# DakeQQ/Text-to-Speech-TTS-ONNX

Measured on AMD Instinct MI355X. Metric: audio_seconds_per_second, higher is better.
Workload: dtype f32

## Files before the change

text-to-speech-tts-onnx_amd/csrc/capi.hip:

```cpp
#include "common.h"
#include "bigvgan.h"
#include "f5.h"
#include "gpt.h"
#include "gpt_pick.h"
#include "cond.h"
#include <algorithm>
#include <mutex>
#include <exception>

using namespace mi;

struct mi_bigvgan { BigVGAN* impl; std::mutex mu; };
struct mi_f5 { F5* impl; std::mutex mu; };
struct mi_gpt { Gpt* impl; std::mutex mu; };
struct mi_cond { Cond* impl; std::mutex mu; };

template <typename F> static int guard(F&& f, bool exclusive = false) {
    try {
        options_init();
        std::shared_lock<std::shared_mutex> rd(option_lock(), std::defer_lock);
        std::unique_lock<std::shared_mutex> wr(option_lock(), std::defer_lock);
        if (exclusive) wr.lock(); else rd.lock();
        f();
        return MI_OK;
// ... 122 lines not shown

int mi_bigvgan_forward_latent(mi_bigvgan* h, const float* latent, int T_codes, const float* conds, int64_t n_conds,
                              int16_t* out, float* out_f32, int mem) {
    return guard([&] {
        MI_REQUIRE(h && h->impl, "mi_bigvgan_forward_latent: null handle");
        std::lock_guard<std::mutex> lk_(h->mu);
        MI_REQUIRE(mem == MI_HOST || mem == MI_DEVICE, "mi_bigvgan_forward_latent: bad mem kind");
        h->impl->run_latent(latent, T_codes, conds, (long)n_conds, out_f32, out, mem);
    });
}

static std::vector<int> bigvgan_lengths(const int64_t* lens, int B, int64_t lo, const char* what) {
    MI_REQUIRE(lens && B >= 1, what);
    std::vector<int> v(B);
    for (int b = 0; b < B; ++b) {
        MI_REQUIRE(lens[b] >= lo && lens[b] < (1L << 30), what);
        v[b] = (int)lens[b];
    }
    return v;
}

int mi_bigvgan_forward_ragged(mi_bigvgan* h, int B, const float* mel, const int64_t* frames, int16_t* out_i16, float* out_f32,
                              int64_t out_cap, int64_t* out_lens, int mem) {
    return guard([&] {
        MI_REQUIRE(h && h->impl, "mi_bigvgan_forward_ragged: null handle");
        std::lock_guard<std::mutex> lk_(h->mu);
        MI_REQUIRE(mem == MI_HOST || mem == MI_DEVICE, "mi_bigvgan_forward_ragged: bad mem kind");
        MI_REQUIRE(out_i16, "mi_bigvgan_forward_ragged: null out_i16");
        const std::vector<int> F = bigvgan_lengths(frames, B, 1, "mi_bigvgan_forward_ragged: B >= 1 items of >= 1 frames");
        h->impl->run_ragged(mel, B, F.data(), out_f32, out_i16, (long)out_cap, out_lens, mem);
    });
}

int mi_bigvgan_forward_latent_ragged(mi_bigvgan* h, int B, const float* latent, const int64_t* t_codes, const float* conds,
                                     int64_t n_conds, int16_t* out_i16, float* out_f32, int64_t out_cap, int64_t* out_lens, int mem) {
    return guard([&] {
        MI_REQUIRE(h && h->impl, "mi_bigvgan_forward_latent_ragged: null handle");
        std::lock_guard<std::mutex> lk_(h->mu);
        MI_REQUIRE(mem == MI_HOST || mem == MI_DEVICE, "mi_bigvgan_forward_latent_ragged: bad mem kind");
        MI_REQUIRE(out_i16, "mi_bigvgan_forward_latent_ragged: null out_i16");
        const std::vector<int> T = bigvgan_lengths(t_codes, B, 3, "mi_bigvgan_forward_latent_ragged: B >= 1 items of >= 3 latent rows");
        h->impl->run_latent_ragged(latent, B, T.data(), conds, (long)n_conds, out_f32, out_i16, (long)out_cap, out_lens, mem);
    });
}

int mi_aa_activation1d(const float* x, int B, int C, int T, const float* alpha_log, const float* beta_log,
                       int logscale, int post, int dtype, float* y) {
    return guard([&] {
        MI_REQUIRE(x && y && alpha_log && beta_log && B > 0 && C > 0 && T > 0, "mi_aa_activation1d: bad arguments");
        unit_aa_activation1d(x, B, C, T, alpha_log, beta_log, logscale, post, dtype, y);
    });
}

int mi_aa_conv1d(const float* x, int B, int C, int T, const float* alpha_log, const float* beta_log, int logscale,
                 const float* w, const float* bias, int k, int dilation, const float* res, int dtype, float* y) {
    return guard([&] {
        MI_REQUIRE(x && y && w && bias && alpha_log && beta_log && B > 0 && C > 0 && T > 0 && k > 0 && (k & 1) && dilation > 0,
                   "mi_aa_conv1d: bad arguments");
        unit_aa_conv1d(x, B, C, T, alpha_log, beta_log, logscale, w, bias, k, dilation, res, dtype, 1, y);
    });
}

int mi_conv1d(const float* x, int B, int Cin, int T, const float* w, const float* bias, int Cout, int k, int dilation,
              int padding, int groups, int dtype, float* y) {
    return guard([&] {
        MI_REQUIRE(x && w && y && B > 0 && Cin > 0 && Cout > 0 && T > 0 && k > 0 && dilation > 0 && groups > 0 && padding >= 0,
                   "mi_conv1d: bad arguments");
        unit_conv1d(x, B, Cin, T, w, bias, Cout, k, dilation, padding, groups, dtype, y);
    });
}

int mi_conv_transpose1d(const float* x, int B, int Cin, int T, const float* w, const float* bias, int Cout, int k,
                        int stride, int padding, int dtype, float* y) {
    return guard([&] {
        MI_REQUIRE(x && w && y && B > 0 && Cin > 0 && Cout > 0 && T > 0, "mi_conv_transpose1d: bad arguments");
        unit_conv_transpose1d(x, B, Cin, T, w, bias, Cout, k, stride, padding, dtype, y);
    });
}

int64_t mi_f5_param_count(const int32_t* cfg_i, int n_i, const float* cfg_f, int n_f) {
    int64_t n = -1;
    int rc = guard([&] { n = f5_param_count(parse_f5_cfg(cfg_i, n_i, cfg_f, n_f)); });
    return rc == MI_OK ? n : (int64_t)rc;
}

mi_f5* mi_f5_create(const int32_t* cfg_i, int n_i, const float* cfg_f, int n_f, const float* weights, int64_t n_weights,
                    int dtype, int device) {
    mi_f5* h = nullptr;
    int rc = guard([&] {
        MI_REQUIRE(weights != nullptr, "mi_f5_create: null weights");
        F5Cfg c = parse_f5_cfg(cfg_i, n_i, cfg_f, n_f);
        F5* impl = new F5(c, weights, n_weights, dtype, device);
        h = new mi_f5; h->impl = impl;
    });
    return rc == MI_OK ? h : nullptr;
}

mi_f5* mi_f5_create_mem(const int32_t* cfg_i, int n_i, const float* cfg_f, int n_f, const float* weights, int64_t n_weights,
                        int dtype, int device, int mem) {
    mi_f5* h = nullptr;
    int rc = guard([&] {
        MI_REQUIRE(weights != nullptr && (mem == MI_HOST || mem == MI_DEVICE), "mi_f5_create_mem: null weights / bad mem kind");
        F5Cfg c = parse_f5_cfg(cfg_i, n_i, cfg_f, n_f);
        F5* impl = new F5(c, weights, n_weights, dtype, device, mem);
        h = new mi_f5; h->impl = impl;
    });
    return rc == MI_OK ? h : nullptr;
}

void mi_f5_destroy(mi_f5* h) {
    if (!h) return;
    delete h->impl;
    delete h;
}

struct F5Recover {
    F5* e; int n;
    explicit F5Recover(F5* e_) : e(e_), n(std::uncaught_exceptions()) {}
    ~F5Recover() { if (std::uncaught_exceptions() > n) e->recover(); }
};
#define F5_CHECK(h, mem, name)                                                     \
    MI_REQUIRE((h) && (h)->impl, name ": null handle");                            \
    std::lock_guard<std::mutex> lk_((h)->mu);                                      \
    F5Recover rec_((h)->impl);                                                     \
    ArithScope arith_((h)->impl->arith);                                           \
    MI_REQUIRE((mem) == MI_HOST || (mem) == MI_DEVICE, name ": bad mem kind")

static void copy_out(void* dst, const void* src, size_t bytes, int mem, hipStream_t s) {
    if (!dst) return;
    MI_HIP(hipMemcpyAsync(dst, src, bytes, mem == MI_HOST ? hipMemcpyDeviceToHost : hipMemcpyDeviceToDevice, s));
}

int mi_f5_tables(mi_f5* h, float* time_expand, float* delta_t) {
    return guard([&] {
        MI_REQUIRE(h && h->impl, "mi_f5_tables: null handle");
        std::lock_guard<std::mutex> lk_(h->mu);
        F5& e = *h->impl;
        if (time_expand) std::memcpy(time_expand, e.h_time_expand.data(), e.h_time_expand.size() * 4);
        if (delta_t) std::memcpy(delta_t, e.h_delta.data(), e.h_delta.size() * 4);
    });
}

int64_t mi_f5_info(mi_f5* h, const char* key) {
    int64_t v = -1;
    int rc = guard([&] {
        MI_REQUIRE(h && h->impl && key, "mi_f5_info: null handle / key");
        std::lock_guard<std::mutex> lk_(h->mu);
        F5& e = *h->impl;
        ArithScope as(e.arith);
        const std::string k(key);
        if (k == "f32_arithmetic") v = e.dtype != MI_F32 ? -1 : !gemm_x3_enabled() ? ARITH_NATIVE : (gemm_x3p_enabled() ? e.np : ARITH_BF16X3);
        else if (k == "saturation_events") v = e.sat_events;
        else if (k == "adaln_fold") v = (e.fold_built && e.cfg.ln_fold != 0) ? 1 : 0;
        else if (k == "attn_v_rows") v = attention_kv_layout(0, e.dtype, true).v_rows;
        else MI_REQUIRE(false, "mi_f5_info: unknown key");
    });
    return rc == MI_OK ? v : (int64_t)rc;
}

int mi_f5_preprocess(mi_f5* h, const int16_t* audio, int64_t L, const int32_t* text_ids, int64_t T, int64_t max_duration,
                     const float* noise_in, uint64_t seed, float* noise, float* rope_cos, float* rope_sin,
                     float* cat_mel_text, float* cat_mel_text_drop, int64_t* ref_signal_len, int mem) {
    return guard([&] {
        F5_CHECK(h, mem, "mi_f5_preprocess");
        F5& e = *h->impl;
        MI_REQUIRE(max_duration > 0 && max_duration <= e.cfg.max_len && T >= 0 && T < (1 << 20) && L > 0 && L < (1L << 31),
                   "mi_f5_preprocess: sizes");
        const int N = (int)max_duration;
        const int R = e.preprocess(1, audio, L, text_ids, (int)T, N, noise_in, seed, mem);
        hipStream_t s = e.stream;
        const size_t cd = e.cfg.cond_dim(), D = e.cfg.dim_head;
        copy_out(noise, e.d_noise.p, (size_t)N * e.cfg.mel * 4, mem, s);
        copy_out(rope_cos, e.rope_cos.p, (size_t)N * D * 4, mem, s);
        copy_out(rope_sin, e.rope_sin.p, (size_t)N * D * 4, mem, s);
        copy_out(cat_mel_text, e.d_cmt.p, (size_t)N * cd * 4, mem, s);
        copy_out(cat_mel_text_drop, e.d_cmtd.p, (size_t)N * cd * 4, mem, s);
        MI_HIP(hipStreamSynchronize(s));
        e.finish_call();
        if (ref_signal_len) *ref_signal_len = R;
    });
}

int mi_f5_transformer_step(mi_f5* h, float* noise, const float* cmt, const float* cmtd, int U, int64_t N,
                           int32_t* time_step, int fuse, int mem) {
    return guard([&] {
        F5_CHECK(h, mem, "mi_f5_transformer_step");
        MI_REQUIRE(noise && cmt && cmtd && time_step && fuse >= 1 && U >= 1 && N > 0, "mi_f5_transformer_step: bad arguments");
        F5& e = *h->impl;
        f5_run_checked(e, [&] {
            e.load_cond(noise, cmt, cmtd, U, (int)N, mem);
            e.build_cat_cond(U, (int)N);
            e.steps(U, (int)N, *time_step, fuse);
            MI_HIP(hipStreamSynchronize(e.stream));
        });
        copy_out(noise, e.d_noise.p, (size_t)U * N * e.cfg.mel * 4, mem, e.stream);
        MI_HIP(hipStreamSynchronize(e.stream));
        e.finish_call();
        *time_step += fuse;
    });
}

int mi_f5_sample(mi_f5* h, float* noise, const float* cmt, const float* cmtd, int U, int64_t N, int k0, int n_steps, int mem) {
    return guard([&] {
        F5_CHECK(h, mem, "mi_f5_sample");
        MI_REQUIRE(noise && cmt && cmtd && U >= 1 && N > 0, "mi_f5_sample: bad arguments");
        F5& e = *h->impl;
        f5_run_checked(e, [&] {
            e.load_cond(noise, cmt, cmtd, U, (int)N, mem);
            e.build_cat_cond(U, (int)N);
            e.steps(U, (int)N, k0, n_steps);
            MI_HIP(hipStreamSynchronize(e.stream));
        });
        copy_out(noise, e.d_noise.p, (size_t)U * N * e.cfg.mel * 4, mem, e.stream);
        MI_HIP(hipStreamSynchronize(e.stream));
        e.finish_call();
    });
}

int mi_f5_dit_eval(mi_f5* h, const float* noise, const float* cmt, const float* cmtd, int U, int64_t N, int k, float* pred, int mem) {
    return guard([&] {
        F5_CHECK(h, mem, "mi_f5_dit_eval");
        MI_REQUIRE(noise && cmt && cmtd && pred && U >= 1 && N > 0, "mi_f5_dit_eval: bad arguments");
        F5& e = *h->impl;
        f5_run_checked(e, [&] {
            e.load_cond(noise, cmt, cmtd, U, (int)N, mem);
            e.build_cat_cond(U, (int)N);
            e.dit_eval(U, (int)N, k);
            MI_HIP(hipStreamSynchronize(e.stream));
        });
        copy_out(pred, e.pred_rows(U, (int)N), (size_t)2 * U * N * e.cfg.mel * 4, mem, e.stream);
        MI_HIP(hipStreamSynchronize(e.stream));
        e.finish_call();
    });
}

int mi_f5_decode(mi_f5* h, const float* denoised, int U, int64_t N, int64_t ref_signal_len, int16_t* out, float* out_f32,
                 int64_t* out_len, int mem) {
    return guard([&] {
        F5_CHECK(h, mem, "mi_f5_decode");
        MI_REQUIRE(denoised && (out || out_f32) && U >= 1 && N > 0 && ref_signal_len >= 0 && ref_signal_len < N,
                   "mi_f5_decode: bad arguments");
        F5& e = *h->impl;
        e.load_cond(denoised, nullptr, nullptr, U, (int)N, mem);
        const long len = e.decode(e.d_noise.as<float>(), U, (int)N, (int)ref_signal_len, out_f32 ? e.v_outf.as<float>() : nullptr,
                                  out ? e.v_outi.as<int16_t>() : nullptr);
        copy_out(out, e.v_outi.p, (size_t)U * len * 2, mem, e.stream);
        copy_out(out_f32, e.v_outf.p, (size_t)U * len * 4, mem, e.stream);
        MI_HIP(hipStreamSynchronize(e.stream));
        e.finish_call();
        if (out_len) *out_len = len;
    });
}

int mi_f5_synthesize(mi_f5* h, int U, const int16_t* audio, int64_t L, const int32_t* text_ids, int64_t T,
                     int64_t max_duration, const float* noise_in, uint64_t seed, int16_t* out, int64_t* out_len, int mem) {
    return guard([&] {
        F5_CHECK(h, mem, "mi_f5_synthesize");
        MI_REQUIRE(audio && text_ids && out && U >= 1 && max_duration > 0, "mi_f5_synthesize: bad arguments");
        F5& e = *h->impl;
        const int N = (int)max_duration;
        long len = 0;
        f5_run_checked(e, [&] {
            const int R = e.preprocess(U, audio, L, text_ids, (int)T, N, noise_in, seed, mem);
            e.build_cat_cond(U, N);
            e.steps(U, N, 0, e.cfg.nfe - 1);
            len = e.decode(e.d_noise.as<float>(), U, N, R, nullptr, e.v_outi.as<int16_t>());
            copy_out(out, e.v_outi.p, (size_t)U * len * 2, mem, e.stream);
            MI_HIP(hipStreamSynchronize(e.stream));
        });
        e.finish_call();
        if (out_len) *out_len = len;
    });
}

int mi_f5_synthesize_mel(mi_f5* h, int U, const int16_t* audio, int64_t L, const int32_t* text_ids, int64_t T,
                         int64_t max_duration, const float* noise_in, uint64_t seed, float* mel_out, int64_t* n_frames, int mem) {
    return guard([&] {
        F5_CHECK(h, mem, "mi_f5_synthesize_mel");
        MI_REQUIRE(audio && text_ids && mel_out && U >= 1 && max_duration > 0, "mi_f5_synthesize_mel: bad arguments");
        F5& e = *h->impl;
        const int N = (int)max_duration;
        int F = 0;
        f5_run_checked(e, [&] {
            const int R = e.preprocess(U, audio, L, text_ids, (int)T, N, noise_in, seed, mem);
            const int mel = e.cfg.mel;
            F = N - R;
            MI_REQUIRE(F >= 1, "mi_f5_synthesize_mel: max_duration leaves no generated frames");
            e.build_cat_cond(U, N);
            e.steps(U, N, 0, e.cfg.nfe - 1);
            float* dst = mel_out;
            if (mem == MI_HOST) { e.v_outf.ensure((size_t)U * mel * F * 4); dst = e.v_outf.as<float>(); }
            for (int u = 0; u < U; ++u)
                launch_nlc_to_ncl(e.d_noise.as<float>() + ((size_t)u * N + R) * mel, dst + (size_t)u * mel * F, 1, mel, F, MI_F32, e.stream);
            if (mem == MI_HOST) copy_out(mel_out, dst, (size_t)U * mel * F * 4, mem, e.stream);
            MI_HIP(hipStreamSynchronize(e.stream));
        });
        e.finish_call();
        if (n_frames) *n_frames = F;
    });
}

static std::vector<int> f5_lengths(const int64_t* lens, int U, int64_t lo, int64_t hi, const char* what) {
    MI_REQUIRE(lens && U >= 1, what);
    std::vector<int> v(U);
    for (int u = 0; u < U; ++u) {
        MI_REQUIRE(lens[u] >= lo && lens[u] <= hi, what);
// ... 930 lines not shown
```

text-to-speech-tts-onnx_amd/csrc/common.h:

```cpp
#pragma once
#include <hip/hip_runtime.h>
#include <hip/hip_fp16.h>
#include <cstdint>
#include <cstdio>
#include <cstring>
#include <cmath>
#include <string>
#include <vector>
#include <stdexcept>
#include <map>
#include <shared_mutex>

#include "../../include/mi355tts.h"
#include "options.h"

namespace mi {

struct Error : std::runtime_error {
    int code;
    Error(int c, const std::string& m) : std::runtime_error(m), code(c) {}
};
void set_last_error(const std::string& m);

#define MI_HIP(expr)                                                                              \
    do {                                                                                          \
        hipError_t _e = (expr);                                                                   \
        if (_e != hipSuccess)                                                                     \
            throw mi::Error(MI_EHIP, std::string(#expr) + ": " + hipGetErrorString(_e) + " @" +   \
                                         __FILE__ + ":" + std::to_string(__LINE__));              \
    } while (0)

#define MI_REQUIRE(cond, msg)                                                                     \
    do {                                                                                          \
        if (!(cond)) throw mi::Error(MI_EINVAL, std::string(msg) + " [" #cond "]");               \
    } while (0)

using f16 = _Float16;
using bf16 = __bf16;
typedef unsigned int u32x4 __attribute__((ext_vector_type(4)));

template <typename T> struct DT;
template <> struct DT<float> { static constexpr int id = MI_F32; };
template <> struct DT<f16>   { static constexpr int id = MI_F16; };
template <> struct DT<bf16>  { static constexpr int id = MI_BF16; };

inline size_t dtype_size(int dt) { return dt == MI_F32 ? 4 : 2; }

template <typename T> __host__ __device__ inline float to_f32(T v) { return (float)v; }
template <typename T> __host__ __device__ inline T from_f32(float v) { return (T)v; }

struct DevBuf {
    void* p = nullptr;
    size_t bytes = 0;
    DevBuf() = default;
    DevBuf(const DevBuf&) = delete;
    DevBuf& operator=(const DevBuf&) = delete;
    DevBuf(DevBuf&& o) noexcept : p(o.p), bytes(o.bytes) { o.p = nullptr; o.bytes = 0; }
    DevBuf& operator=(DevBuf&& o) noexcept {
        if (this != &o) { release(); p = o.p; bytes = o.bytes; o.p = nullptr; o.bytes = 0; }
        return *this;
    }
    ~DevBuf() { release(); }
    void release() { if (p) { (void)hipFree(p); p = nullptr; bytes = 0; } }
    void ensure(size_t n) {
        if (n <= bytes) return;
        release();
        MI_HIP(hipMalloc(&p, n));
        bytes = n;
    }
    template <typename T> T* as() const { return reinterpret_cast<T*>(p); }
};

void upload_as(DevBuf& dst, const float* src, size_t n, int dt, hipStream_t s);
void upload_f32(DevBuf& dst, const float* src, size_t n, hipStream_t s);
int device_cus();

struct BlobReader {
    int mem; hipStream_t s;
    std::vector<std::vector<float>> keep;
    BlobReader(int mem_, hipStream_t s_) : mem(mem_), s(s_) {}
    const float* host(const float* p, size_t n);
    void put(DevBuf& dst, const float* p, size_t n, int dt, size_t dst_off = 0);
};

struct ProfScope {
    int fam; hipStream_t s; hipEvent_t e0 = nullptr, e1 = nullptr; bool on; double bytes_ = 0, flops_ = 0;
    ProfScope(int family, hipStream_t stream, double bytes, double flops);
    ~ProfScope();
};
enum { FAM_CONV_GEMM = 0, FAM_AA = 1, FAM_CONV_POST = 2, FAM_ATTN = 3, FAM_NORM = 4, FAM_OTHER = 5, FAM_COUNT = 6 };
void prof_set_kernel(const char* expr, const char* t = nullptr, const char* to = nullptr);
void prof_kernel_suffix(const char* sfx);
template <typename T> inline const char* type_label();
template <> inline const char* type_label<float>() { return "float"; }
template <> inline const char* type_label<f16>() { return "_Float16"; }
template <> inline const char* type_label<bf16>() { return "__bf16"; }
#define MI_LAUNCH(K, T_, TO_, grid, blk, lds, s, ...)                                                  \
    do {                                                                                               \
        mi::prof_set_kernel(#K, mi::type_label<T_>(), mi::type_label<TO_>());                          \
        hipLaunchKernelGGL(K, grid, blk, lds, s, __VA_ARGS__);                                         \
    } while (0)
void prof_collect();
unsigned prof_mask();

enum Act { ACT_NONE = 0, ACT_GELU_TANH = 1, ACT_GELU_ERF = 2, ACT_MISH = 3, ACT_SILU = 4 };
enum EpiMode { EPI_PLAIN = 0, EPI_CONVT = 1, EPI_QKV_ROPE = 2 };

struct ConvGemm {
    int dtype = MI_F32;
    int out_dtype = -1;
    const void* x = nullptr;
    const void* w = nullptr;
    const float* bias = nullptr;
    void* out = nullptr;
    const void* res = nullptr;
    const float* gate = nullptr;
    long gate_bstride = 0;
    int B = 1, G = 1;
    int T_in = 0;
    int M = 0, N = 0, Cin = 0, taps = 1, dil = 1, pad = 0;
    long x_bstride = 0, x_rstride = 0;
    long out_bstride = 0, out_rstride = 0;
    long x_goff = 0;
    int act = ACT_NONE;
    float alpha = 1.f;
    int accumulate = 0;
    int epi = EPI_PLAIN;
    int u = 1, Cout = 0, padT = 0, T_out = 0;
    const float* rope_cos = nullptr; const float* rope_sin = nullptr; int heads = 0, head_dim = 0;
    const void* rope_pack = nullptr;
    void* out2 = nullptr; void* out3 = nullptr;
    int rows_per_item = 0;
    int m_off = 0;
    long v_ld = 0;
    int kv_planes = 0; long k_ld = 0;
    int v_rows = 0;
    float* sk_ws = nullptr; int* sk_flags = nullptr; int sk_slots = 0;
    const void* w3 = nullptr;
    const void* xp = nullptr; const void* w3p = nullptr; int np = 3;
    const void* gcp_w = nullptr;
    void* out_planes = nullptr;
    const float* ln_scale = nullptr; void* ln_out = nullptr; float* ln_stats_out = nullptr; int ln_out_np = 0;
    const float* ln_stats_in = nullptr; const float* ln_p = nullptr; const float* ln_c = nullptr; int ln_dim = 0; float ln_eps = 0.f;
    int ln_final = 0;
    int* sat = nullptr;
    const int* lens = nullptr; int len_mul = 1, len_add = 0;
};
constexpr int LN_BLK = 32;
void launch_conv_gemm(const ConvGemm& p, hipStream_t s);
bool gemm_ln_fold_ok(const ConvGemm& p);
constexpr int X3P_PLANE = 128 * 32 * 2;
constexpr int X3P_CHUNK = 3 * X3P_PLANE;
__host__ __device__ inline int x3p_chunk_bytes(int np) { return np * X3P_PLANE; }
__host__ __device__ inline long x3p_slot_offset(long row, int s8, int nch, int np = 3) {
    const int r = (int)(row & 127);
    return ((row >> 7) * nch + (s8 >> 2)) * (long)(np * X3P_PLANE) + r * 64 + (((s8 & 3) ^ ((r >> 2) & 3)) << 4);
}
long x3p_bytes(long rows, long K, int np = 3);
void x3p_split_rows(const float* x, long ld, void* planes, int rows, int K, hipStream_t s, int np = 3, int* sat = nullptr);
size_t gconv_pairs_planes_bytes(int G, int taps);
void gconv_pairs_split_weights(const float* w, void* wp, int G, int taps, hipStream_t s);
size_t gconv16_image_bytes(int G, int taps);
void gconv16_build_weights(const void* w, int dtype, void* img, int G, int taps, hipStream_t s);
int x3p_planes();
bool gemm_x3p_enabled();
bool gemm_x3p_would_run(const ConvGemm& p);
bool gemm_x3p_can_write_planes(const ConvGemm& p);
struct SkWorkspace {
    DevBuf ws, flags; int slots = 0;
    void ensure(int n_slots, hipStream_t s);
    void reset(hipStream_t s);
    bool tripped() const;
    void attach(ConvGemm& g) const { g.sk_ws = ws.as<float>(); g.sk_flags = flags.as<int>(); g.sk_slots = slots; }
};

struct ArithOverride {
    int gemm_x3 = -1;
    int gemm_x3p = -1;
    int planes = -1;
    int n64_pairs = -1;
    int gconv = -1;
    int attn_x3 = -1;
    int attn_np = -1;
};
enum { ARITH_DEFAULT = -1, ARITH_NATIVE = 0, ARITH_PAIRS = 2, ARITH_BF16X3 = 3 };
ArithOverride arith_for(int kind);
ArithOverride& arith_tls();
struct ArithScope {
    ArithOverride saved;
    explicit ArithScope(const ArithOverride& a) : saved(arith_tls()) { arith_tls() = a; }
    ~ArithScope() { arith_tls() = saved; }
    ArithScope(const ArithScope&) = delete;
    ArithScope& operator=(const ArithScope&) = delete;
};

struct AAAct {
    int dtype = MI_F32;
    const void* x = nullptr; void* y = nullptr;
    const float* alpha = nullptr;
    const float* inv_beta = nullptr;
    int B = 1, T = 0, C = 0;
    int post = 0;
    const int* lens = nullptr; int len_mul = 1, len_add = 0;
};
void launch_aa_act(const AAAct& p, hipStream_t s);
const float* aa_filter_host();

struct AAConv {
    int dtype = MI_F32;
    const void* x = nullptr; const void* w = nullptr;
    const float* bias = nullptr;
    const float* snake_alpha = nullptr; const float* snake_inv_beta = nullptr;
    void* out = nullptr; const void* res = nullptr;
    int B = 1, T = 0, C = 0, k = 3, dil = 1;
    float alpha = 1.f; int accumulate = 0;
    const int* lens = nullptr; int len_mul = 1, len_add = 0;
};
void launch_aa_conv(const AAConv& p, hipStream_t s);
void split3_planes(const float* w, void* planes, long n, hipStream_t s);
bool gemm_x3_enabled();

void launch_ncl_to_nlc(const float* x, void* y, int B, int C, int T, int Cpad, int dtype, hipStream_t s);
void launch_ncl_to_nlc_len(const float* x, void* y, int B, int C, int T, int Cpad, int dtype, const int* lens, const long* offs,
                           hipStream_t s);
void launch_nlc_to_ncl(const void* x, float* y, int B, int C, int T, int dtype, hipStream_t s);
void launch_conv_post(const void* x, const float* w , float bias, int B, int T, int C, int dtype,
                      int use_tanh, float* out_f32, int16_t* out_i16, hipStream_t s);
void launch_conv_post_len(const void* x, const float* w, float bias, int B, int T, int C, int dtype, int use_tanh, float* out_f32,
                          int16_t* out_i16, const int* lens, int len_mul, int len_add, const long* offs, hipStream_t s);

}
```

text-to-speech-tts-onnx_amd/csrc/f5.h:

```cpp
#pragma once
#include <algorithm>

#include "common.h"
#include "f5_kernels.h"

namespace mi {

struct F5Cfg {
    int dim, depth, heads, dim_head, ff_mult, mel, text_dim, vocab, conv_layers, conv_mult, pos_k, pos_g, freq_dim,
        nfe, max_len, n_fft, hop, sr, vd, vi, vlayers;
    float cfg_strength, sway;
    float score_scale = 1.f;
    int f32_arith = ARITH_DEFAULT;
    int mel_type = 0;
    int ln_fold = -1;
    int ff() const { return dim * ff_mult; }
    int nb() const { return n_fft / 2 + 1; }
    int cat_dim() const { return 2 * mel + text_dim; }
    int cond_dim() const { return mel + text_dim; }
};
F5Cfg parse_f5_cfg(const int32_t* ci, int ni, const float* cf, int nf);
int64_t f5_param_count(const F5Cfg& c);

struct Lin { DevBuf w, b, w3, w3p; int n = 0, k = 0; };

struct F5 {
    F5Cfg cfg;
    int dtype, device;
    hipStream_t stream = nullptr;

    Lin in_proj, gconv1, gconv2, proj_out;
    Lin proj_out_k; int proj_parts = 1; DevBuf pred_sum;
    const float* pred_rows(int U, int N);
    int cat_pad = 0;
    int cat_ld() const { return cfg.cat_dim() + cat_pad; }
    struct Block { Lin qkv, o, ff1, ff2; };
    std::vector<Block> blocks;
    DevBuf mod;
    long mod_ld = 0;
    DevBuf delta_t;
    DevBuf rope_cos, rope_sin;
    DevBuf rope_pack;
    std::vector<float> h_time_expand, h_delta;

    DevBuf text_emb, text_pos, stft_w, fbank;
    struct TextBlock { DevBuf dw_w, dw_b, ln_w, ln_b, grn_g, grn_b; Lin pw1, pw2; };
    std::vector<TextBlock> tblocks;

    Lin v_embed, v_head, istft;
    DevBuf v_norm_w, v_norm_b, v_fnorm_w, v_fnorm_b, wsi;
    struct VBlock { DevBuf dw_w, dw_b, n_w, n_b; Lin pw1, pw2; };
    std::vector<VBlock> vblocks;

    struct GraphEntry { hipGraphExec_t exec = nullptr; int uses = 0; };
    std::map<std::vector<int>, GraphEntry> graphs;
    bool use_graph = true;
    long graph_epoch = 0;
    void drop_graphs();
    void recover();
    void steps_eager(int U, int N, int k0, int nsteps, const int* lens = nullptr);

    SkWorkspace sk;
    DevBuf attn_ws, attn_cnt;
    long attn_ws_floats = 0, attn_cnt_n = 0;
    int ws_U = 0, ws_N = 0;
    int np = 3;
    ArithOverride arith;
    int arith_kind = ARITH_DEFAULT;
    DevBuf Ap, Ap2;
    int ap2_cols() const { return std::max(cfg.ff(), cat_ld()); }
    bool fold_built = false;
    DevBuf ApN;
    DevBuf ln_stats;
    DevBuf ln_fin;
    DevBuf ln_tab;
    long ln_ld = 0, ln_blk = 0;
    DevBuf d_sat;
    long sat_events = 0;
    void build_ln_tables(int i, DevBuf& G, DevBuf& S, DevBuf& tmpw);
    void set_arith(int kind);
    bool take_saturation();
    void finish_call();
    DevBuf d_noise, d_cmt, d_cmtd, cat, h32, hT, c1, X, Ub, qb, kb, vb, Ob, Hff, pred;
    DevBuf p_audio, p_pad, p_spec, p_mag, p_mel, p_ids, p_tid, p_err, p_tx, p_ty, p_ty2, p_ss;
    std::vector<float> h_noise;
    DevBuf v_h, v_z, v_z2, v_s, v_c, v_fr, v_outf, v_outi;

    F5(const F5Cfg& c, const float* w, int64_t nw, int dt, int dev, int mem = MI_HOST);
    ~F5();
    void ensure_workspace(int U, int N);
    void gemm(int dt, const void* x, long xb, long xr, int K, const Lin& L, void* out, int odt, long ob, long orr,
              int B, int M, int act = ACT_NONE, const void* res = nullptr, const float* gate = nullptr);
    int preprocess(int U, const int16_t* audio, long L, const int32_t* text_ids, int T, int N,
                   const float* noise_in, uint64_t seed, int mem);
    void stft(const int16_t* audio_dev, int U, long L, int pad = -1);
    void check_text_ids();
    void load_cond(const float* noise, const float* cmt, const float* cmtd, int U, int N, int mem);
    void build_cat_cond(int U, int N);
    void dit_eval(int U, int N, int k, const int* lens = nullptr);
    void steps(int U, int N, int k0, int nsteps, const int* lens = nullptr);
    DevBuf d_len;
    std::vector<int> h_len;
    int ref_frames(long L) const;
    const int* set_lengths(int U, const int* lens);
    void zero_pad_rows_cond(int U, int Nmax, const int* lens);
    void preprocess_ragged(int U, const int16_t* audio, const long* L, const int32_t* text_ids, const int* T, const int* Ns, int Nmax,
                           const float* noise_in, uint64_t seed, int mem, int* R);
    long decode(const float* denoised_dev, int U, int N, int R, float* out_f, int16_t* out_i);
};

}
```

text-to-speech-tts-onnx_amd/csrc/f5.hip:

```cpp
#include "f5.h"

namespace mi {

static int rup(int a, int b) { return (a + b - 1) / b * b; }

F5Cfg parse_f5_cfg(const int32_t* ci, int ni, const float* cf, int nf) {
    MI_REQUIRE(ci && ni >= 21 && ni <= 24 && cf && (nf == 2 || nf == 3),
               "f5 cfg: expected 21 ints (+ up to 3 optional: fp32 arithmetic, mel type, AdaLN fold) + 2 floats (+ the optional attention score scale)");
    F5Cfg c;
    int i = 0;
    c.dim = ci[i++]; c.depth = ci[i++]; c.heads = ci[i++]; c.dim_head = ci[i++]; c.ff_mult = ci[i++]; c.mel = ci[i++];
    c.text_dim = ci[i++]; c.vocab = ci[i++]; c.conv_layers = ci[i++]; c.conv_mult = ci[i++]; c.pos_k = ci[i++];
    c.pos_g = ci[i++]; c.freq_dim = ci[i++]; c.nfe = ci[i++]; c.max_len = ci[i++]; c.n_fft = ci[i++]; c.hop = ci[i++];
    c.sr = ci[i++]; c.vd = ci[i++]; c.vi = ci[i++]; c.vlayers = ci[i++];
    if (ni > 21) c.f32_arith = ci[21];
    if (ni > 22) c.mel_type = ci[22];
    if (ni > 23) c.ln_fold = ci[23];
    MI_REQUIRE(c.f32_arith == ARITH_DEFAULT || c.f32_arith == ARITH_NATIVE || c.f32_arith == ARITH_PAIRS || c.f32_arith == ARITH_BF16X3,
               "f5 cfg: fp32 arithmetic is -1 (process default), 0 (native fp32 MFMA), 2 (fp16 pairs) or 3 (three bf16 planes)");
    MI_REQUIRE((c.mel_type == 0 || c.mel_type == 1) && c.ln_fold >= -1 && c.ln_fold <= 1, "f5 cfg: mel type is 0 (vocos) or 1 (bigvgan); AdaLN fold is -1, 0 or 1");
    c.cfg_strength = cf[0]; c.sway = cf[1];
    if (nf == 3) { c.score_scale = cf[2]; MI_REQUIRE(c.score_scale > 0.f && c.score_scale <= 1e4f, "f5 cfg: attention score scale"); }
    MI_REQUIRE(c.dim == c.heads * c.dim_head, "f5 cfg: dim != heads*dim_head");
    MI_REQUIRE(c.dim_head == 64, "f5: the attention kernel is built for head_dim 64");
    MI_REQUIRE(c.dim % 32 == 0 && c.dim <= 2048 && c.text_dim % 8 == 0 && c.mel % 4 == 0, "f5 cfg: widths");
    MI_REQUIRE(c.dim % c.pos_g == 0 && (c.dim / c.pos_g) % 8 == 0 && c.pos_k % 2 == 1, "f5 cfg: pos conv");
    MI_REQUIRE(c.nfe >= 2 && c.nfe <= 1024 && c.max_len >= 16 && c.depth > 0, "f5 cfg: sampler");
    MI_REQUIRE(c.n_fft % 8 == 0 && c.n_fft % c.hop == 0 && c.vd % 4 == 0 && c.vi % 4 == 0 && c.vd <= 2048, "f5 cfg: vocoder");
    MI_REQUIRE(c.freq_dim % 2 == 0 && c.conv_mult >= 1 && c.text_dim * c.conv_mult <= 4096, "f5 cfg: text");
    return c;
}

int64_t f5_param_count(const F5Cfg& c) {
    const int64_t d = c.dim, td = c.text_dim, ff = c.ff(), ti = td * c.conv_mult, cin = c.cat_dim();
    int64_t n = d * c.freq_dim + d + d * d + d;
    n += (int64_t)(c.vocab + 1) * td;
    n += (int64_t)c.conv_layers * (td * 7 + td + td + td + ti * td + ti + ti + ti + td * ti + td);
    n += d * cin + d + 2 * (d * (d / c.pos_g) * c.pos_k + d);
    n += (int64_t)c.depth * (6 * d * d + 6 * d + 4 * (d * d + d) + ff * d + ff + d * ff + d);
    n += 2 * d * d + 2 * d + (int64_t)c.mel * d + c.mel;
    const int64_t vd = c.vd, vi = c.vi;
    n += vd * c.mel * 7 + vd + 2 * vd;
    n += (int64_t)c.vlayers * (vd * 7 + vd + 2 * vd + vi * vd + vi + vd * vi + vd);
    n += 2 * vd + (int64_t)(c.n_fft + 2) * vd + (c.n_fft + 2);
    return n;
}

static void up_lin(Lin& L, const float* w, const float* b, int n, int k, int dt, hipStream_t s) {
    L.n = n; L.k = k;
    upload_as(L.w, w, (size_t)n * k, dt, s);
    if (b) upload_f32(L.b, b, n, s);
}
static void put_lin(BlobReader& R, Lin& L, const float* w, const float* b, int n, int k, int dt) {
    L.n = n; L.k = k;
    R.put(L.w, w, (size_t)n * k, dt);
    if (b) R.put(L.b, b, n, MI_F32);
}
static std::vector<float> relayout(const float* w, int Co, int Ci, int k) {
    std::vector<float> o((size_t)Co * k * Ci);
    for (int co = 0; co < Co; ++co)
        for (int ci = 0; ci < Ci; ++ci)
            for (int j = 0; j < k; ++j) o[((size_t)co * k + j) * Ci + ci] = w[((size_t)co * Ci + ci) * k + j];
    return o;
}
static inline float siluf(float v) { return v / (1.f + expf(-v)); }
static inline float round_f16(float v) { return (float)(f16)v; }

F5::F5(const F5Cfg& c, const float* w, int64_t nw, int dt, int dev, int mem) : cfg(c), dtype(dt), device(dev) {
    arith_kind = dt == MI_F32 ? c.f32_arith : ARITH_DEFAULT;
    arith = arith_for(arith_kind);
    ArithScope arith_scope(arith);
    np = x3p_planes();
    MI_REQUIRE(dt == MI_F32 || dt == MI_F16 || dt == MI_BF16, "f5: bad dtype");
    MI_REQUIRE(c.score_scale == 1.f || dt == MI_F16, "f5: the attention score scale (reference fp16-transformer form) needs an f16 engine");
    MI_REQUIRE(nw == f5_param_count(c), "f5: weight blob size does not match the config");
    MI_HIP(hipSetDevice(dev));
    MI_HIP(hipStreamCreateWithFlags(&stream, hipStreamNonBlocking));
    use_graph = !env_first_is("MI355TTS_NO_GRAPH", '1');
    hipStream_t s = stream;
    d_sat.ensure(64);
    MI_HIP(hipMemsetAsync(d_sat.p, 0, 64, s));
    const int d = c.dim, td = c.text_dim, ff = c.ff(), ti = td * c.conv_mult, cin = c.cat_dim();
    if (dt == MI_F32 && !env_first_is("MI355TTS_CAT_PAD", '0')) cat_pad = rup(cin, 64) - cin;
    const float* p = w;
    auto take = [&](size_t n) { const float* r = p; p += n; return r; };
    BlobReader R(mem, s);

    const float* tw0 = R.host(take((size_t)d * c.freq_dim), (size_t)d * c.freq_dim); const float* tb0 = R.host(take(d), d);
    const float* tw2 = R.host(take((size_t)d * d), (size_t)d * d); const float* tb2 = R.host(take(d), d);
    const int steps = c.nfe, half = c.freq_dim / 2;
    std::vector<float> ts(steps);
    for (int i = 0; i < steps; ++i) {
        const float t = (float)i / (float)(steps - 1);
        ts[i] = t + c.sway * (cosf(3.14159265358979323846f * 0.5f * t) - 1.f + t);
    }
    h_delta.resize(steps - 1);
    for (int i = 0; i + 1 < steps; ++i) h_delta[i] = ts[i + 1] - ts[i];
    upload_f32(delta_t, h_delta.data(), steps - 1, s);
    h_time_expand.assign((size_t)steps * d, 0.f);
    {
        const float ef = logf(10000.f) / (float)(half - 1);
        std::vector<float> emb(c.freq_dim), hid(d);
        for (int i = 0; i < steps; ++i) {
            for (int j = 0; j < half; ++j) {
                const float a = ts[i] * (1000.0f * expf((float)j * -ef));
                emb[j] = sinf(a); emb[half + j] = cosf(a);
            }
            for (int o = 0; o < d; ++o) {
                float acc = tb0[o];
                for (int j = 0; j < c.freq_dim; ++j) acc += tw0[(size_t)o * c.freq_dim + j] * emb[j];
                hid[o] = siluf(acc);
            }
            for (int o = 0; o < d; ++o) {
                float acc = tb2[o];
                for (int j = 0; j < d; ++j) acc += tw2[(size_t)o * d + j] * hid[j];
                h_time_expand[(size_t)i * d + o] = acc;
            }
        }
    }
    R.put(text_emb, take((size_t)(c.vocab + 1) * td), (size_t)(c.vocab + 1) * td, MI_F32);
    {
        std::vector<float> pos((size_t)c.max_len * td);
        std::vector<float> fr(td / 2);
        for (int j = 0; j < td / 2; ++j) fr[j] = 1.0f / powf(10000.0f, (float)(2 * j) / (float)td);
        for (int n = 0; n < c.max_len; ++n)
            for (int j = 0; j < td / 2; ++j) {
                const float a = (float)n * fr[j];
                pos[(size_t)n * td + j] = cosf(a); pos[(size_t)n * td + td / 2 + j] = sinf(a);
            }
        upload_f32(text_pos, pos.data(), pos.size(), s);
    }
    tblocks.resize(c.conv_layers);
    for (auto& tb : tblocks) {
        R.put(tb.dw_w, take((size_t)td * 7), (size_t)td * 7, MI_F32);
        R.put(tb.dw_b, take(td), td, MI_F32);
        R.put(tb.ln_w, take(td), td, MI_F32);
        R.put(tb.ln_b, take(td), td, MI_F32);
        const float* w1 = take((size_t)ti * td); const float* b1 = take(ti);
        put_lin(R, tb.pw1, w1, b1, ti, td, MI_F32);
        R.put(tb.grn_g, take(ti), ti, MI_F32);
        R.put(tb.grn_b, take(ti), ti, MI_F32);
        const float* w2 = take((size_t)td * ti); const float* b2 = take(td);
        put_lin(R, tb.pw2, w2, b2, td, ti, MI_F32);
    }
    {
        const float* pw = take((size_t)d * cin); const float* pb = take(d);
        if (cat_ld() == cin) put_lin(R, in_proj, pw, pb, d, cin, dt);
        else {
            const int kp = cat_ld();
            const float* hw = R.host(pw, (size_t)d * cin); const float* hb = R.host(pb, d);
            std::vector<float> wp((size_t)d * kp, 0.f);
            for (int o = 0; o < d; ++o) std::copy(hw + (size_t)o * cin, hw + (size_t)(o + 1) * cin, wp.begin() + (size_t)o * kp);
            up_lin(in_proj, wp.data(), hb, d, kp, dt, s);
        }
        const int cg = d / c.pos_g;
        const size_t gw = (size_t)d * cg * c.pos_k;
        const float* w1 = R.host(take(gw), gw); const float* b1 = R.host(take(d), d);
        auto r1 = relayout(w1, d, cg, c.pos_k);
        up_lin(gconv1, r1.data(), b1, d, cg * c.pos_k, dt, s);
        const float* w2 = R.host(take(gw), gw); const float* b2 = R.host(take(d), d);
        auto r2 = relayout(w2, d, cg, c.pos_k);
        up_lin(gconv2, r2.data(), b2, d, cg * c.pos_k, dt, s);
        if (dt != MI_F32 && cg == 64 && c.pos_k >= 8 && c.pos_k <= 127) {
            for (Lin* L : {&gconv1, &gconv2}) {
                L->w3p.ensure(gconv16_image_bytes(c.pos_g, c.pos_k));
                gconv16_build_weights(L->w.p, dt, L->w3p.p, c.pos_g, c.pos_k, s);
            }
        }
        if (dt == MI_F32 && cg == 64 && c.pos_k >= 8 && c.pos_k <= 127) {
            for (Lin* L : {&gconv1, &gconv2}) {
                L->w3p.ensure(gconv_pairs_planes_bytes(c.pos_g, c.pos_k));
                gconv_pairs_split_weights(L->w.as<float>(), L->w3p.p, c.pos_g, c.pos_k, s);
            }
        }
    }
    mod_ld = (long)c.depth * 6 * d + 2 * d;
    mod.ensure((size_t)steps * mod_ld * 4);
    DevBuf d_silu_t, d_tmpw, d_tmpb;
    {
        std::vector<float> st(h_time_expand.size());
        for (size_t i = 0; i < st.size(); ++i) st[i] = siluf(h_time_expand[i]);
        upload_f32(d_silu_t, st.data(), st.size(), s);
    }
    auto mod_gemm = [&](const float* mw, const float* mb, int n, long col) {
        R.put(d_tmpw, mw, (size_t)n * d, MI_F32);
        R.put(d_tmpb, mb, n, MI_F32);
        ConvGemm g;
        g.dtype = MI_F32; g.x = d_silu_t.p; g.w = d_tmpw.p; g.bias = d_tmpb.as<float>(); g.out = mod.as<float>() + col;
        g.B = 1; g.T_in = steps; g.M = steps; g.N = n; g.Cin = d; g.x_rstride = d; g.x_bstride = (long)steps * d;
        g.out_rstride = mod_ld; g.out_bstride = (long)steps * mod_ld;
        launch_conv_gemm(g, s);
        MI_HIP(hipStreamSynchronize(s));
    };
    blocks.resize(c.depth);
    for (int i = 0; i < c.depth; ++i) {
        Block& bk = blocks[i];
        const float* mw = take((size_t)6 * d * d); const float* mb = take((size_t)6 * d);
        mod_gemm(mw, mb, 6 * d, (long)i * 6 * d);
        bk.qkv.n = 3 * d; bk.qkv.k = d;
        bk.qkv.w.ensure((size_t)3 * d * d * dtype_size(dt)); bk.qkv.b.ensure((size_t)3 * d * 4);
        for (int t3 = 0; t3 < 3; ++t3) {
            const float* wt = take((size_t)d * d); const float* bt = take(d);
            if (t3 == 0) { R.put(bk.qkv.w, wt, (size_t)d * d, dt, 0); R.put(bk.qkv.b, bt, d, MI_F32, 0); }
            else { R.put(bk.qkv.w, wt, (size_t)d * d, dt, (size_t)t3 * d * d); R.put(bk.qkv.b, bt, d, MI_F32, (size_t)t3 * d); }
        }
        const float* wo = take((size_t)d * d); const float* bo = take(d);
        put_lin(R, bk.o, wo, bo, d, d, dt);
        const float* w1 = take((size_t)ff * d); const float* b1 = take(ff);
        put_lin(R, bk.ff1, w1, b1, ff, d, dt);
        const float* w2 = take((size_t)d * ff); const float* b2 = take(d);
        put_lin(R, bk.ff2, w2, b2, d, ff, dt);
        if (dt == MI_F32) {
            for (Lin* L : {&bk.qkv, &bk.o, &bk.ff1, &bk.ff2}) {
                L->w3.ensure((size_t)3 * L->n * L->k * 2);
                split3_planes(L->w.as<float>(), L->w3.p, (long)L->n * L->k, s);
                launch_absmax(L->w.as<float>(), (long)L->n * L->k, d_sat.as<unsigned>() + 1, s);
            }
        }
    }
    if (dt == MI_F32) {
        unsigned bits = 0;
        MI_HIP(hipMemcpyAsync(&bits, d_sat.as<unsigned>() + 1, 4, hipMemcpyDeviceToHost, s));
        MI_HIP(hipStreamSynchronize(s));
        float wmax; std::memcpy(&wmax, &bits, 4);
        int kind = arith_kind;
        if (np == 2 && gemm_x3p_enabled() && !(wmax < 65504.f)) kind = ARITH_BF16X3;
        set_arith(kind);
    }
    fold_built = false;
    const bool want_fold = c.ln_fold != 0;
    if (want_fold && d >= 1024 && d % 128 == 0 && ff % 64 == 0) {
        ln_blk = (long)6 * d + 2 * ff;
        ln_ld = (long)c.depth * ln_blk;
        ln_tab.ensure((size_t)steps * ln_ld * 4);
        DevBuf G, S, tmpw;
        G.ensure((size_t)steps * d * 4); S.ensure((size_t)steps * d * 4);
        if (dt != MI_F32) tmpw.ensure((size_t)std::max(3 * d, ff) * d * 4);
        for (int i = 0; i < c.depth; ++i) build_ln_tables(i, G, S, tmpw);
        MI_HIP(hipStreamSynchronize(s));
        fold_built = true;
    }
    {
        const float* mw = take((size_t)2 * d * d); const float* mb = take((size_t)2 * d);
        mod_gemm(mw, mb, 2 * d, (long)c.depth * 6 * d);
        const float* pw = take((size_t)c.mel * d); const float* pb = take(c.mel);
        put_lin(R, proj_out, pw, pb, c.mel, d, dt);
        {
            const int parts = (int)env_int("MI355TTS_PROJ_PARTS", 4);
            if (dt == MI_F32 && parts > 1 && parts <= 8 && d % (parts * 32) == 0) {
                proj_parts = parts;
                const int kq = d / parts;
                const float* hw = R.host(pw, (size_t)c.mel * d); const float* hb = R.host(pb, c.mel);
                std::vector<float> wq((size_t)c.mel * d), bq((size_t)parts * c.mel, 0.f);
                for (int q = 0; q < parts; ++q)
                    for (int o = 0; o < c.mel; ++o)
                        std::copy(hw + (size_t)o * d + (size_t)q * kq, hw + (size_t)o * d + (size_t)(q + 1) * kq, wq.begin() + ((size_t)q * c.mel + o) * kq);
                std::copy(hb, hb + c.mel, bq.begin());
                up_lin(proj_out_k, wq.data(), bq.data(), parts * c.mel, kq, dt, s);
            }
        }
    }
    {
        const int D = c.dim_head;
        std::vector<float> rc((size_t)c.max_len * D), rs((size_t)c.max_len * D);
        for (int n = 0; n < c.max_len; ++n)
            for (int j = 0; j < D / 2; ++j) {
                const float inv = 1.0f / powf(10000.0f, (float)(2 * j) / (float)D);
                const float a = (float)n * inv;
                const float cc = round_f16(cosf(a)), ss = round_f16(sinf(a));
                rc[(size_t)n * D + 2 * j] = rc[(size_t)n * D + 2 * j + 1] = cc;
                rs[(size_t)n * D + 2 * j] = rs[(size_t)n * D + 2 * j + 1] = ss;
            }
        upload_f32(rope_cos, rc.data(), rc.size(), s);
        upload_f32(rope_sin, rs.data(), rs.size(), s);
        std::vector<f16> pk((size_t)c.max_len * D);
        for (int n = 0; n < c.max_len; ++n)
            for (int j = 0; j < D / 2; ++j) {
                pk[(size_t)n * D + 2 * j] = (f16)rc[(size_t)n * D + 2 * j];
                pk[(size_t)n * D + 2 * j + 1] = (f16)rs[(size_t)n * D + 2 * j];
            }
        rope_pack.ensure(pk.size() * sizeof(f16));
        MI_HIP(hipMemcpyAsync(rope_pack.p, pk.data(), pk.size() * sizeof(f16), hipMemcpyHostToDevice, s));
        MI_HIP(hipStreamSynchronize(s));
    }
    {
        const int nf = c.n_fft, nb = c.nb();
        std::vector<float> win(nf);
        const float wstep = (float)(2.0 * M_PI / nf);
        for (int n = 0; n < nf; ++n) win[n] = cosf((float)n * wstep) * -0.5f + 0.5f;
        std::vector<float> sw((size_t)2 * nb * nf);
        const float two_pi = (float)(2.0 * M_PI);
        for (int f = 0; f < nb; ++f)
            for (int t = 0; t < nf; ++t) {
                const float om = ((two_pi * (float)f) * (float)t) / (float)nf;
                sw[(size_t)f * nf + t] = cosf(om) * win[t];
                sw[(size_t)(nb + f) * nf + t] = -sinf(om) * win[t];
            }
        if (c.mel_type == 1) {
            for (int f = 0; f < nb; ++f)
                for (int t = 0; t < nf; ++t) {
                    const double om = 2.0 * M_PI * (double)((long)f * t % nf) / nf;
                    sw[(size_t)f * nf + t] = (float)(std::cos(om) * (double)win[t]);
                    sw[(size_t)(nb + f) * nf + t] = (float)(-std::sin(om) * (double)win[t]);
                }
        }
        upload_f32(stft_w, sw.data(), sw.size(), s);
        const int ldm = rup(nb, 8);
        std::vector<float> fb((size_t)c.mel * ldm, 0.f);
        if (c.mel_type == 1) {
            const double f_sp = 200.0 / 3, min_log_hz = 1000.0, logstep = std::log(6.4) / 27.0, min_log_mel = min_log_hz / f_sp;
            auto h2m = [&](double f) { return f < min_log_hz ? f / f_sp : min_log_mel + std::log(f / min_log_hz) / logstep; };
            auto m2h = [&](double m) { return m < min_log_mel ? f_sp * m : min_log_hz * std::exp(logstep * (m - min_log_mel)); };
            const double m0 = h2m(0.0), m1 = h2m((double)c.sr / 2);
            std::vector<double> mf(c.mel + 2);
            for (int i = 0; i < c.mel + 2; ++i) mf[i] = m2h(m0 + (m1 - m0) * i / (c.mel + 1));
            for (int m = 0; m < c.mel; ++m) {
                const double enorm = 2.0 / (mf[m + 2] - mf[m]);
                for (int k = 0; k < nb; ++k) {
                    const double fr = (double)c.sr / 2 * k / (nb - 1);
                    const double lower = (fr - mf[m]) / (mf[m + 1] - mf[m]), upper = (mf[m + 2] - fr) / (mf[m + 2] - mf[m + 1]);
                    fb[(size_t)m * ldm + k] = (float)(std::max(0.0, std::min(lower, upper)) * enorm);
                }
            }
        }
        const double m_min = 0.0, m_max = 2595.0 * std::log10(1.0 + (c.sr / 2) / 700.0);
        std::vector<double> fpts(c.mel + 2);
        for (int i = 0; i < c.mel + 2; ++i) {
            const double m = m_min + (m_max - m_min) * i / (c.mel + 1);
            fpts[i] = 700.0 * (std::pow(10.0, m / 2595.0) - 1.0);
        }
        for (int k = 0; k < nb && c.mel_type == 0; ++k) {
            const double fr = (double)(c.sr / 2) * k / (nb - 1);
            for (int m = 0; m < c.mel; ++m) {
                const double down = (fr - fpts[m]) / (fpts[m + 1] - fpts[m]);
                const double up = (fpts[m + 2] - fr) / (fpts[m + 2] - fpts[m + 1]);
                fb[(size_t)m * ldm + k] = (float)std::max(0.0, std::min(down, up));
            }
        }
        upload_f32(fbank, fb.data(), fb.size(), s);
        const int kp = rup(2 * nb, 4);
        std::vector<float> ib((size_t)nf * kp, 0.f);
        for (int n = 0; n < nf; ++n)
            for (int k = 0; k < nb; ++k) {
                const double sc = ((k == 0 || k == nb - 1) ? 1.0 : 2.0) / nf * ((double)c.hop / nf) * (double)win[n];
                const double ang = 2.0 * M_PI * (double)k * (double)n / nf;
                ib[(size_t)n * kp + k] = (float)(sc * std::cos(ang));
                ib[(size_t)n * kp + nb + k] = (float)(sc * -std::sin(ang));
            }
        istft.n = nf; istft.k = kp;
        upload_f32(istft.w, ib.data(), ib.size(), s);
        const size_t wl = (size_t)nf + (size_t)c.hop * (c.max_len - 1);
        std::vector<float> ws(wl, 0.f);
        float wmax = 0.f;
        for (int n = 0; n < nf; ++n) wmax = std::max(wmax, fabsf(win[n]));
        std::vector<float> wsq(nf);
        for (int n = 0; n < nf; ++n) { const float wn = win[n] / wmax; wsq[n] = wn * wn; }
        for (int i = 0; i < c.max_len; ++i)
            for (int n = 0; n < nf; ++n) ws[(size_t)i * c.hop + n] += wsq[n];
        for (size_t i = 0; i < wl; ++i) ws[i] = (float)nf / (ws[i] * (float)c.hop + 1e-7f);
        upload_f32(wsi, ws.data(), wl, s);
    }
    {
        const int vd = c.vd, vi = c.vi;
        const size_t ewn = (size_t)vd * c.mel * 7;
        const float* ew = R.host(take(ewn), ewn); const float* eb = R.host(take(vd), vd);
        auto re = relayout(ew, vd, c.mel, 7);
        up_lin(v_embed, re.data(), eb, vd, c.mel * 7, MI_F32, s);
        R.put(v_norm_w, take(vd), vd, MI_F32); R.put(v_norm_b, take(vd), vd, MI_F32);
        vblocks.resize(c.vlayers);
        for (auto& vb_ : vblocks) {
            R.put(vb_.dw_w, take((size_t)vd * 7), (size_t)vd * 7, MI_F32); R.put(vb_.dw_b, take(vd), vd, MI_F32);
            R.put(vb_.n_w, take(vd), vd, MI_F32); R.put(vb_.n_b, take(vd), vd, MI_F32);
            const float* w1 = take((size_t)vi * vd); const float* b1 = take(vi);
            put_lin(R, vb_.pw1, w1, b1, vi, vd, MI_F32);
            const float* w2 = take((size_t)vd * vi); const float* b2 = take(vd);
            put_lin(R, vb_.pw2, w2, b2, vd, vi, MI_F32);
        }
        R.put(v_fnorm_w, take(vd), vd, MI_F32); R.put(v_fnorm_b, take(vd), vd, MI_F32);
        const float* hw = take((size_t)(c.n_fft + 2) * vd); const float* hb = take(c.n_fft + 2);
        put_lin(R, v_head, hw, hb, c.n_fft + 2, vd, MI_F32);
    }
    MI_HIP(hipStreamSynchronize(s));
    MI_REQUIRE(p - w == nw, "f5: weight walk mismatch");
}

F5::~F5() {
    drop_graphs();
    if (stream) (void)hipStreamDestroy(stream);
}

void F5::set_arith(int kind) {
    arith_kind = kind;
    arith = arith_for(kind);
    ArithScope sc(arith);
    np = x3p_planes();
    drop_graphs();
    if (dtype != MI_F32) return;
    const bool planes = gemm_x3p_enabled();
    auto build_planes = [&](Lin* L) {
        if (!planes || L->n % 128 != 0 || L->k % 32 != 0) { L->w3p.release(); return; }
        L->w3p.ensure((size_t)x3p_bytes(L->n, L->k, np));
        x3p_split_rows(L->w.as<float>(), L->k, L->w3p.p, L->n, L->k, stream, np);
    };
    for (Block& bk : blocks)
        for (Lin* L : {&bk.qkv, &bk.o, &bk.ff1, &bk.ff2}) build_planes(L);
    build_planes(&in_proj);
    if (ws_U > 0) {
        const long rows = (long)2 * ws_U * ws_N;
        Ap.ensure((size_t)x3p_bytes(rows, cfg.dim, np)); Ap2.ensure((size_t)x3p_bytes(rows, ap2_cols(), np)); ApN.ensure((size_t)x3p_bytes(rows, cfg.dim, np));
    }
    MI_HIP(hipStreamSynchronize(stream));
}

void F5::build_ln_tables(int i, DevBuf& G, DevBuf& S, DevBuf& tmpw) {
    const int d = cfg.dim, ff = cfg.ff(), steps = cfg.nfe;
    Block& bk = blocks[i];
    float* tab = ln_tab.as<float>() + (size_t)i * ln_blk;
    auto run = [&](const Lin& L, long col_shift, long col_scale, float* out_p, float* out_c) {
        launch_ln_gather(mod.as<float>(), mod_ld, (long)i * 6 * d + col_scale, (long)i * 6 * d + col_shift, G.as<float>(), S.as<float>(), steps, d, stream);
        const float* w32 = L.w.as<float>();
        if (dtype != MI_F32) { launch_cast_to_f32(L.w.p, dtype, tmpw.as<float>(), (long)L.n * L.k, stream); w32 = tmpw.as<float>(); }
        ConvGemm g;
        g.dtype = MI_F32; g.x = G.p; g.w = w32; g.bias = nullptr; g.out = out_p;
        g.B = 1; g.T_in = steps; g.M = steps; g.N = L.n; g.Cin = d; g.x_rstride = d; g.x_bstride = (long)steps * d;
        g.out_rstride = ln_ld; g.out_bstride = (long)steps * ln_ld;
        launch_conv_gemm(g, stream);
        g.x = S.p; g.bias = L.b.as<float>(); g.out = out_c;
        launch_conv_gemm(g, stream);
        MI_HIP(hipStreamSynchronize(stream));
    };
    run(bk.qkv, 0, d, tab, tab + 3 * d);
    run(bk.ff1, 3 * d, 4 * d, tab + 6 * d, tab + 6 * d + ff);
}

bool F5::take_saturation() {
    if (!d_sat.p) return false;
    int flag = 0;
    MI_HIP(hipMemcpy(&flag, d_sat.p, 4, hipMemcpyDeviceToHost));
    if (!flag) return false;
    MI_HIP(hipMemset(d_sat.p, 0, 4));
    return true;
}

void F5::finish_call() {
    check_text_ids();
}

void F5::ensure_workspace(int U, int N) {
    if (U <= ws_U && N <= ws_N) return;
    drop_graphs();
    const int Um = std::max(U, ws_U), Nm = std::max(N, ws_N);
    const F5Cfg& c = cfg;
    const size_t es = dtype_size(dtype);
    const size_t rows = (size_t)2 * Um * Nm;
    sk.ensure(1024, stream);
    {
        if (ATTN_WS_TILES > attn_cnt_n) {
            attn_ws_floats = ATTN_WS_TILES * ATTN_MAX_SLICES * ATTN_SLOT_SPLIT;
            attn_ws.ensure((size_t)attn_ws_floats * 4);
            attn_cnt.ensure((size_t)ATTN_WS_TILES * 4);
            MI_HIP(hipMemsetAsync(attn_cnt.p, 0, (size_t)ATTN_WS_TILES * 4, stream));
            attn_cnt_n = ATTN_WS_TILES;
        }
    }
    d_noise.ensure((size_t)Um * Nm * c.mel * 4);
    d_cmt.ensure((size_t)Um * Nm * c.cond_dim() * 4);
    d_cmtd.ensure((size_t)Um * Nm * c.cond_dim() * 4);
    if (rows * cat_ld() * es > cat.bytes) {
        cat.ensure(rows * cat_ld() * es);
        if (cat_ld() != c.cat_dim()) MI_HIP(hipMemsetAsync(cat.p, 0, cat.bytes, stream));
    }
    h32.ensure(rows * c.dim * 4); hT.ensure(rows * c.dim * es); c1.ensure(rows * c.dim * es);
    X.ensure(rows * c.dim * 4); Ub.ensure(rows * c.dim * es);
    qb.ensure(rows * c.dim * es); Ob.ensure(rows * c.dim * es);
    {
        const size_t keypad = (size_t)(Nm + 63) / 64 * 64;
        size_t kbytes = rows * c.dim * es, vbytes = (size_t)2 * Um * (size_t)(Nm + 8) * c.dim * es;
        if (dtype == MI_F32) { kbytes = std::max(kbytes, (size_t)2 * Um * keypad * c.dim * 6); vbytes = std::max(vbytes, (size_t)2 * Um * keypad * c.dim * 6); }
        if (kbytes > kb.bytes) { kb.ensure(kbytes); MI_HIP(hipMemsetAsync(kb.p, 0, kbytes, stream)); }
        if (vbytes > vb.bytes) { vb.ensure(vbytes); MI_HIP(hipMemsetAsync(vb.p, 0, vbytes, stream)); }
    }
    Hff.ensure(rows * c.ff() * es);
    if (dtype == MI_F32) {
        Ap.ensure((size_t)x3p_bytes((long)rows, c.dim, np)); Ap2.ensure((size_t)x3p_bytes((long)rows, ap2_cols(), np));
        if (fold_built) ApN.ensure((size_t)x3p_bytes((long)rows, c.dim, np));
    }
    if (fold_built) { ln_stats.ensure((rows + 128) * (size_t)(c.dim / LN_BLK) * 2 * 4); if (dtype != MI_F32) ln_fin.ensure((rows + 128) * 8); }
    pred.ensure(rows * c.mel * 4 * proj_parts);
    if (proj_parts > 1) pred_sum.ensure(rows * c.mel * 4);
    const int ti = c.text_dim * c.conv_mult;
    p_ids.ensure((size_t)Um * Nm * 4);
    p_tx.ensure((size_t)2 * Um * Nm * c.text_dim * 4); p_ty.ensure((size_t)2 * Um * Nm * c.text_dim * 4);
    p_ty2.ensure((size_t)2 * Um * Nm * ti * 4); p_ss.ensure((size_t)2 * Um * ti * 4);
    const size_t fr = (size_t)Um * Nm;
    v_h.ensure(fr * c.vd * 4); v_z.ensure(fr * c.vd * 4); v_z2.ensure(fr * c.vi * 4);
    v_s.ensure(fr * (c.n_fft + 2) * 4); v_c.ensure(fr * istft.k * 4); v_fr.ensure(fr * c.n_fft * 4);
    v_outf.ensure(fr * c.hop * 4); v_outi.ensure(fr * c.hop * 2);
    ws_U = Um; ws_N = Nm;
}

void F5::gemm(int dt, const void* x, long xb, long xr, int K, const Lin& L, void* out, int odt, long ob, long orr, int B,
              int M, int act, const void* res, const float* gate) {
    ConvGemm g;
    g.dtype = dt; g.out_dtype = odt; g.x = x; g.w = L.w.p; g.w3 = L.w3.p; g.bias = L.b.p ? L.b.as<float>() : nullptr; g.out = out;
    g.res = res; g.gate = gate; g.gate_bstride = 0;
    g.B = B; g.T_in = M; g.M = M; g.N = L.n; g.Cin = K; g.taps = 1;
    g.x_bstride = xb; g.x_rstride = xr; g.out_bstride = ob; g.out_rstride = orr; g.act = act;
    g.sat = d_sat.as<int>();
    sk.attach(g);
    if (B > 1 && xb == (long)M * xr && ob == (long)M * orr) {
        g.B = 1; g.T_in = B * M; g.M = B * M;
    }
    if (dt == MI_F32 && L.w3p.p && g.B == 1 && Ap.p && gemm_x3p_enabled()) {
        DevBuf& ab = K <= cfg.dim ? Ap : Ap2;
        g.xp = ab.p; g.w3p = L.w3p.p; g.np = np;
        if (gemm_x3p_would_run(g)) {
            MI_REQUIRE(x3p_bytes(g.M, K, np) <= (long)ab.bytes, "F5::gemm: the panel planes of the rows do not fit their buffer");
            x3p_split_rows((const float*)x, xr, const_cast<void*>(g.xp), g.M, K, stream, np, d_sat.as<int>());
        } else {
            g.xp = nullptr; g.w3p = nullptr;
        }
    }
    launch_conv_gemm(g, stream);
}

static inline uint64_t splitmix64(uint64_t x) {
    x += 0x9E3779B97F4A7C15ull;
    uint64_t z = x;
    z = (z ^ (z >> 30)) * 0xBF58476D1CE4E5B9ull;
    z = (z ^ (z >> 27)) * 0x94D049BB133111EBull;
    return z ^ (z >> 31);
}
static void host_normal(float* out, size_t n, uint64_t seed) {
    for (size_t i = 0; i < n; ++i) {
        const uint64_t a = splitmix64(seed * 0x2545F4914F6CDD1Dull + 2 * i), b = splitmix64(seed * 0x2545F4914F6CDD1Dull + 2 * i + 1);
        const double u1 = ((double)(a >> 11) + 1.0) / 9007199254740993.0, u2 = (double)(b >> 11) / 9007199254740992.0;
        out[i] = (float)(std::sqrt(-2.0 * std::log(u1)) * std::cos(2.0 * M_PI * u2));
    }
}

int F5::preprocess(int U, const int16_t* audio, long L, const int32_t* text_ids, int T, int N,
                   const float* noise_in, uint64_t seed, int mem) {
    const F5Cfg& c = cfg;
    MI_REQUIRE(audio && text_ids && U >= 1 && L >= c.n_fft / 2 + 1 && T >= 0, "f5_preprocess: bad arguments");
    const int mel_pad = c.mel_type == 1 ? (c.n_fft - c.hop) / 2 : c.n_fft / 2;
    MI_REQUIRE(L + 2 * mel_pad >= c.n_fft && L > mel_pad, "f5_preprocess: audio shorter than one STFT frame");
    const int R = (int)((L + 2 * mel_pad - c.n_fft) / c.hop) + 1;
    MI_REQUIRE(N >= R && N >= T && N <= c.max_len, "f5_preprocess: max_duration must be >= ref frames, >= text length and <= max_signal_length");
    if (mem == MI_HOST)
        for (long i = 0; i < (long)U * T; ++i) {
            const long id = (long)text_ids[i] + 1;
            MI_REQUIRE(id >= 0 && id <= c.vocab, "f5_preprocess: text id out of range");
        }
    MI_HIP(hipSetDevice(device));
    ensure_workspace(U, N);
    hipStream_t s = stream;
    const int nf = c.n_fft, nb = c.nb(), ldm = rup(nb, 8), cd = c.cond_dim();
    const long Lp = L + nf;
    p_audio.ensure((size_t)U * L * 2); p_pad.ensure((size_t)U * Lp * 4 + 64);
    p_spec.ensure((size_t)U * R * 2 * nb * 4); p_mag.ensure((size_t)U * R * ldm * 4); p_mel.ensure((size_t)U * R * c.mel * 4);
    p_tid.ensure((size_t)U * std::max(T, 1) * 4); p_err.ensure(4);
    const int16_t* da = audio;
    const int32_t* dt_ids = text_ids;
    if (mem == MI_HOST) {
        MI_HIP(hipMemcpyAsync(p_audio.p, audio, (size_t)U * L * 2, hipMemcpyHostToDevice, s));
        da = p_audio.as<int16_t>();
        if (T > 0) MI_HIP(hipMemcpyAsync(p_tid.p, text_ids, (size_t)U * T * 4, hipMemcpyHostToDevice, s));
        dt_ids = p_tid.as<int32_t>();
    }
    MI_HIP(hipMemsetAsync(p_err.p, 0, 4, s));
    stft(da, U, L, mel_pad);
    launch_spec_mag(p_spec.as<float>(), p_mag.as<float>(), U * R, nb, ldm, c.mel_type == 1 ? 1e-9f : 0.f, s);
    {
        ConvGemm g;
        g.dtype = MI_F32; g.x = p_mag.p; g.w = fbank.p; g.out = p_mel.p;
        g.B = 1; g.T_in = U * R; g.M = U * R; g.N = c.mel; g.Cin = ldm; g.x_rstride = ldm; g.out_rstride = c.mel;
        launch_conv_gemm(g, s);
    }
    launch_logmel(p_mel.as<float>(), d_cmt.as<float>(), d_cmtd.as<float>(), U, N, R, c.mel, cd, s);
    const int td = c.text_dim, ti = td * c.conv_mult;
    int* dids = p_ids.as<int>();
    launch_text_ids(dt_ids, dids, U, T, N, c.vocab, p_err.as<int>(), s);
    float* tx = p_tx.as<float>(); float* ty = p_ty.as<float>(); float* ty2 = p_ty2.as<float>();
    launch_text_gather(dids, text_emb.as<float>(), text_pos.as<float>(), tx, U, N, td, s);
    const int B2 = 2 * U;
    for (auto& tb : tblocks) {
        launch_dwconv7(tx, ty, tb.dw_w.as<float>(), tb.dw_b.as<float>(), B2, N, td, s);
        launch_rownorm(NORM_LN_AFFINE, ty, ty, MI_F32, tb.ln_w.as<float>(), tb.ln_b.as<float>(), (long)B2 * N, td, 1e-6f, s);
        gemm(MI_F32, ty, (long)N * td, td, td, tb.pw1, ty2, MI_F32, (long)N * ti, ti, B2, N, ACT_GELU_ERF);
        launch_grn(ty2, p_ss.as<float>(), tb.grn_g.as<float>(), tb.grn_b.as<float>(), B2, N, ti, s);
        gemm(MI_F32, ty2, (long)N * ti, ti, ti, tb.pw2, tx, MI_F32, (long)N * td, td, B2, N, ACT_NONE, tx);
        launch_mask_rows(dids, tx, B2, N, td, s);
    }
    for (int u = 0; u < U; ++u) {
        launch_copy2d(tx + (size_t)(2 * u) * N * td, td, d_cmt.as<float>() + (size_t)u * N * cd + c.mel, cd, N, td, MI_F32, s);
        launch_copy2d(tx + (size_t)(2 * u + 1) * N * td, td, d_cmtd.as<float>() + (size_t)u * N * cd + c.mel, cd, N, td, MI_F32, s);
    }
    const size_t nn = (size_t)N * c.mel;
    if (noise_in) {
        MI_HIP(hipMemcpyAsync(d_noise.p, noise_in, (size_t)U * nn * 4, mem == MI_HOST ? hipMemcpyHostToDevice : hipMemcpyDeviceToDevice, s));
    } else {
        h_noise.resize((size_t)U * nn);
        for (int u = 0; u < U; ++u) host_normal(h_noise.data() + (size_t)u * nn, nn, seed + (uint64_t)u);
        MI_HIP(hipMemcpyAsync(d_noise.p, h_noise.data(), h_noise.size() * 4, hipMemcpyHostToDevice, s));
    }
    return R;
}

void F5::stft(const int16_t* audio_dev, int U, long L, int pad) {
    const F5Cfg& c = cfg;
    if (pad < 0) pad = c.n_fft / 2;
    const int nf = c.n_fft, nb = c.nb(), R = (int)((L + 2 * pad - nf) / c.hop) + 1;
    const long Lp = L + 2 * pad;
    launch_pad_reflect(audio_dev, p_pad.as<float>(), U, L, pad, stream);
    ConvGemm g;
    g.dtype = MI_F32; g.x = p_pad.p; g.w = stft_w.p; g.out = p_spec.p;
    g.B = U; g.T_in = R; g.M = R; g.N = 2 * nb; g.Cin = nf; g.x_rstride = c.hop; g.x_bstride = Lp;
    g.out_rstride = 2 * nb; g.out_bstride = (long)R * 2 * nb;
    launch_conv_gemm(g, stream);
}

void F5::check_text_ids() {
    if (sk.tripped()) {
        recover();
        MI_REQUIRE(false, "f5: a split-tile hand-off timed out on the device (workspace reset; results of this call discarded)");
    }
    if (!p_err.p) return;
    int flag = 0;
    MI_HIP(hipMemcpy(&flag, p_err.p, 4, hipMemcpyDeviceToHost));
    if (flag != 0) {
        MI_HIP(hipMemset(p_err.p, 0, 4));
        MI_REQUIRE(false, "f5_preprocess: text id out of range");
    }
}

void F5::load_cond(const float* noise, const float* cmt, const float* cmtd, int U, int N, int mem) {
    const F5Cfg& c = cfg;
    MI_REQUIRE(U > 0 && N > 0 && N <= c.max_len, "f5: bad batch / length");
    MI_HIP(hipSetDevice(device));
    ensure_workspace(U, N);
    const hipMemcpyKind kind = mem == MI_HOST ? hipMemcpyHostToDevice : hipMemcpyDeviceToDevice;
    if (noise && noise != d_noise.p) MI_HIP(hipMemcpyAsync(d_noise.p, noise, (size_t)U * N * c.mel * 4, kind, stream));
    if (cmt && cmt != d_cmt.p) MI_HIP(hipMemcpyAsync(d_cmt.p, cmt, (size_t)U * N * c.cond_dim() * 4, kind, stream));
    if (cmtd && cmtd != d_cmtd.p) MI_HIP(hipMemcpyAsync(d_cmtd.p, cmtd, (size_t)U * N * c.cond_dim() * 4, kind, stream));
}

void F5::build_cat_cond(int U, int N) {
    const F5Cfg& c = cfg;
    const size_t es = dtype_size(dtype);
    const int cd = c.cond_dim(), ld = cat_ld();
    for (int u = 0; u < U; ++u)
        for (int br = 0; br < 2; ++br) {
            const float* src = (br == 0 ? d_cmt.as<float>() : d_cmtd.as<float>()) + (size_t)u * N * cd;
            char* dst = (char*)cat.p + ((size_t)(2 * u + br) * N * ld + c.mel) * es;
            launch_copy2d(src, cd, dst, ld, N, cd, dtype, stream);
        }
}

void F5::dit_eval(int U, int N, int k, const int* lens) {
    const F5Cfg& c = cfg;
    MI_REQUIRE(k >= 0 && k < c.nfe, "f5: time step out of range");
    hipStream_t s = stream;
    const int B = 2 * U, d = c.dim, ld = cat_ld(), ff = c.ff(), H = c.heads, D = c.dim_head;
    const long rows = (long)B * N;
    const float* modk = mod.as<float>() + (size_t)k * mod_ld;
    launch_cat_noise(d_noise.as<float>(), cat.p, U, N, c.mel, ld, dtype, s);
    gemm(dtype, cat.p, (long)N * ld, ld, ld, in_proj, h32.p, MI_F32, (long)N * d, d, B, N);
    const void* hin = h32.p;
    if (dtype != MI_F32) { launch_copy2d(h32.as<float>(), d, hT.p, d, rows, d, dtype, s); hin = hT.p; }
    const long row_bytes = (long)d * (long)dtype_size(dtype);
    if (lens) launch_zero_pad_rows(const_cast<void*>(hin), row_bytes, B, N, lens, 2, s);
    {
        ConvGemm g;
        g.dtype = dtype; g.x = hin; g.w = gconv1.w.p; g.bias = gconv1.b.as<float>(); g.out = c1.p;
        g.B = B; g.G = c.pos_g; g.T_in = N; g.M = N; g.N = d / c.pos_g; g.Cin = d / c.pos_g; g.taps = c.pos_k; g.pad = c.pos_k / 2;
        g.x_bstride = (long)N * d; g.x_rstride = d; g.x_goff = d / c.pos_g; g.out_bstride = (long)N * d; g.out_rstride = d;
        g.act = ACT_MISH; g.sat = d_sat.as<int>(); g.gcp_w = gconv1.w3p.p;
        launch_conv_gemm(g, s);
        if (lens) launch_zero_pad_rows(c1.p, row_bytes, B, N, lens, 2, s);
        g.x = c1.p; g.w = gconv2.w.p; g.bias = gconv2.b.as<float>(); g.out = X.p; g.out_dtype = MI_F32; g.res = h32.p; g.gcp_w = gconv2.w3p.p;
        launch_conv_gemm(g, s);
    }
    const bool f32 = dtype == MI_F32;
    auto lin = [&](const Lin& L, int K, int odt, void* out) {
        ConvGemm g;
        g.dtype = dtype; g.out_dtype = odt; g.w = L.w.p; g.w3 = L.w3.p; g.bias = L.b.p ? L.b.as<float>() : nullptr; g.out = out;
        g.B = 1; g.T_in = (int)rows; g.M = (int)rows; g.N = L.n; g.Cin = K; g.taps = 1;
        g.x_bstride = rows * K; g.x_rstride = K; g.out_bstride = rows * L.n; g.out_rstride = L.n;
        g.sat = d_sat.as<int>();
        sk.attach(g);
        return g;
    };
    auto with_planes = [&](ConvGemm& g, const Lin& L, const void* xp) { g.xp = xp; g.w3p = L.w3p.p; g.np = np; };
    auto attn_plan = [&](bool presplit) {
        return attention_plan(B * H, H, N, dtype, presplit, lens != nullptr, cfg.score_scale != 1.f ? cfg.score_scale : 0.f, attn_ws_floats, attn_cnt_n);
    };
    AttnPlan ap = attn_plan(false);
    auto qkv_gemm = [&](const Block& bk) {
        ConvGemm g = lin(bk.qkv, d, -1, qb.p);
        g.x = Ub.p; g.out2 = kb.p; g.out3 = vb.p; g.rows_per_item = N;
        g.epi = EPI_QKV_ROPE; g.rope_cos = rope_cos.as<float>(); g.rope_sin = rope_sin.as<float>(); g.rope_pack = rope_pack.p; g.heads = H; g.head_dim = D;
        g.kv_planes = ap.kv.kv_planes; g.k_ld = ap.kv.k_ld; g.v_ld = ap.kv.v_ld; g.v_rows = ap.kv.v_rows;
        return g;
    };
    bool planes = false, fold = false;
    {
        const Block& b0 = blocks[0];
        ConvGemm gq = qkv_gemm(b0);
        ConvGemm go = lin(b0.o, d, MI_F32, X.p); go.x = Ob.p; go.res = X.p; go.gate = modk;
        ConvGemm g1 = lin(b0.ff1, d, dtype, Hff.p); g1.x = Ub.p; g1.act = ACT_GELU_TANH;
        ConvGemm g2 = lin(b0.ff2, ff, MI_F32, X.p); g2.x = Hff.p; g2.res = X.p; g2.gate = modk;
        if (f32 && Ap.p && gemm_x3p_enabled() && b0.qkv.w3p.p && b0.o.w3p.p && b0.ff1.w3p.p && b0.ff2.w3p.p && ap.o_planes) {
            with_planes(gq, b0.qkv, Ap.p); with_planes(go, b0.o, Ap.p); with_planes(g1, b0.ff1, Ap.p); with_planes(g2, b0.ff2, Ap2.p);
            planes = gemm_x3p_would_run(gq) && gemm_x3p_would_run(go) && gemm_x3p_can_write_planes(g1) && gemm_x3p_would_run(g2);
        }
        if (fold_built && cfg.ln_fold != 0 && (planes || !f32) && (!f32 || ApN.p) && ln_stats.p && (f32 || ln_fin.p)) {
            if (f32) { with_planes(gq, b0.qkv, ApN.p); with_planes(g1, b0.ff1, ApN.p); }
            fold = gemm_ln_fold_ok(gq) && gemm_ln_fold_ok(go) && gemm_ln_fold_ok(g1) && gemm_ln_fold_ok(g2);
        }
    }
    if (f32 && (fold || planes)) ap = attn_plan(true);
    void* const attn_planes = f32 && (fold || planes) ? Ap.p : nullptr;
    auto attention = [&] {
        launch_attention(ap, qb.p, kb.p, vb.p, Ob.p, attn_planes, np, attn_ws.as<float>(), attn_cnt.as<int>(), lens, s);
    };
    float* stats = ln_stats.as<float>();
    const float* lnk = fold ? ln_tab.as<float>() + (size_t)k * ln_ld : nullptr;
    const bool fin = fold && !f32;
    auto finalize = [&] { if (fin) launch_ln_finalize(stats, ln_fin.as<float>(), rows, d, 1e-6f, s); };
    auto consume = [&](ConvGemm& g, const float* p, const float* c_) {
        g.bias = nullptr; g.ln_p = p; g.ln_c = c_;
        g.ln_stats_in = fin ? ln_fin.as<float>() : stats; g.ln_final = fin ? 1 : 0; g.ln_dim = d; g.ln_eps = 1e-6f;
    };
    auto produce = [&](ConvGemm& g, const float* scale) { g.ln_scale = scale; g.ln_out = f32 ? ApN.p : Ub.p; g.ln_out_np = np; g.ln_stats_out = stats; };
    if (fold) {
        launch_ln_prologue(X.as<float>(), f32 ? ApN.p : Ub.p, dtype, np, stats, modk + d, rows, d, d_sat.as<int>(), s);
        finalize();
    }
    const void* normed = fold ? ApN.p : Ap.p;
    auto layer = [&](ConvGemm& g, const Lin& L, const void* xp, const char* left) {
        if (f32) { with_planes(g, L, xp); MI_REQUIRE(gemm_x3p_would_run(g), left); }
        launch_conv_gemm(g, s);
    };
    for (int i = 0; i < c.depth; ++i) {
        const Block& bk = blocks[i];
        const float* m = modk + (size_t)i * 6 * d;
        if (fold || planes) {
            const float* lt = fold ? lnk + (size_t)i * ln_blk : nullptr;
            const bool last = i + 1 == c.depth;
            if (!fold) launch_rownorm_x3p(X.as<float>(), Ap.p, m + d, m, rows, d, 1e-6f, s, np, d_sat.as<int>());
            {
                ConvGemm g = qkv_gemm(bk);
                if (fold) consume(g, lt, lt + 3 * d);
                layer(g, bk.qkv, normed, "f5: the QKV layer left the panel-plane kernel between the decision and the launch");
            }
            attention();
            {
                ConvGemm g = lin(bk.o, d, MI_F32, X.p);
                g.x = Ob.p; g.res = X.p; g.gate = m + 2 * d;
                if (fold) produce(g, m + 4 * d);
                layer(g, bk.o, Ap.p, "f5: the O projection left the panel-plane kernel between the decision and the launch");
                finalize();
            }
            if (!fold) launch_rownorm_x3p(X.as<float>(), Ap.p, m + 4 * d, m + 3 * d, rows, d, 1e-6f, s, np, d_sat.as<int>());
            {
                ConvGemm g = lin(bk.ff1, d, dtype, Hff.p);
                g.x = Ub.p; g.act = ACT_GELU_TANH;
                if (f32) g.out_planes = Ap2.p;
                if (fold) consume(g, lt + 6 * d, lt + 6 * d + ff);
                layer(g, bk.ff1, normed, "f5: the FF1 layer left the panel-plane kernel between the decision and the launch");
            }
            {
                ConvGemm g = lin(bk.ff2, ff, MI_F32, X.p);
                g.x = Hff.p; g.res = X.p; g.gate = m + 5 * d;
                if (fold && !last) produce(g, m + 6 * d + d);
                layer(g, bk.ff2, Ap2.p, "f5: the FF2 layer left the panel-plane kernel between the decision and the launch");
                if (!last) finalize();
            }
            continue;
        }
        launch_rownorm(NORM_LN_MOD, X.as<float>(), Ub.p, dtype, m + d, m, rows, d, 1e-6f, s);
        {
            ConvGemm g = qkv_gemm(bk);
            g.x_bstride = (long)B * N * d;
            launch_conv_gemm(g, s);
        }
        attention();
        gemm(dtype, Ob.p, (long)N * d, d, d, bk.o, X.p, MI_F32, (long)N * d, d, B, N, ACT_NONE, X.p, m + 2 * d);
        launch_rownorm(NORM_LN_MOD, X.as<float>(), Ub.p, dtype, m + 4 * d, m + 3 * d, rows, d, 1e-6f, s);
        gemm(dtype, Ub.p, (long)N * d, d, d, bk.ff1, Hff.p, dtype, (long)N * ff, ff, B, N, ACT_GELU_TANH);
        gemm(dtype, Hff.p, (long)N * ff, ff, ff, bk.ff2, X.p, MI_F32, (long)N * d, d, B, N, ACT_NONE, X.p, m + 5 * d);
    }
    const float* mf = modk + (size_t)c.depth * 6 * d;
    launch_rownorm(NORM_LN_MOD, X.as<float>(), Ub.p, dtype, mf, mf + d, rows, d, 1e-6f, s);
    if (proj_parts > 1) {
        ConvGemm g;
        g.dtype = dtype; g.out_dtype = MI_F32; g.x = Ub.p; g.w = proj_out_k.w.p; g.bias = proj_out_k.b.as<float>(); g.out = pred.p;
        g.B = 1; g.G = proj_parts; g.T_in = (int)rows; g.M = (int)rows; g.N = c.mel; g.Cin = d / proj_parts; g.taps = 1;
        g.x_bstride = rows * d; g.x_rstride = d; g.x_goff = d / proj_parts;
        g.out_bstride = rows * proj_parts * c.mel; g.out_rstride = (long)proj_parts * c.mel;
        launch_conv_gemm(g, s);
    } else
        gemm(dtype, Ub.p, (long)N * d, d, d, proj_out, pred.p, MI_F32, (long)N * c.mel, c.mel, B, N);
}

const float* F5::pred_rows(int U, int N) {
    if (proj_parts <= 1) return pred.as<float>();
    launch_sum_parts(pred.as<float>(), pred_sum.as<float>(), (long)2 * U * N, cfg.mel, proj_parts, stream);
    return pred_sum.as<float>();
}

void F5::steps_eager(int U, int N, int k0, int nsteps, const int* lens) {
    for (int k = k0; k < k0 + nsteps; ++k) {
        dit_eval(U, N, k, lens);
        if (lens)
            launch_cfg_update_len(d_noise.as<float>(), pred.as<float>(), U, N, cfg.mel, cfg.cfg_strength, delta_t.as<float>(), k, lens, stream,
                                  proj_parts);
        else
            launch_cfg_update(d_noise.as<float>(), pred.as<float>(), U, N, cfg.mel, cfg.cfg_strength, delta_t.as<float>(), k, stream, proj_parts);
    }
}

void F5::drop_graphs() {
    for (auto& kv : graphs)
        if (kv.second.exec) (void)hipGraphExecDestroy(kv.second.exec);
    graphs.clear();
}

void F5::recover() {
    (void)hipSetDevice(device);
    (void)hipStreamSynchronize(stream);
    (void)hipGetLastError();
    drop_graphs();
    sk.reset(stream);
    if (attn_cnt.p && attn_cnt_n > 0) {
        (void)hipMemsetAsync(attn_cnt.p, 0, (size_t)attn_cnt_n * 4, stream);
        (void)hipStreamSynchronize(stream);
    }
    if (p_err.p) (void)hipMemset(p_err.p, 0, 4);
    if (d_sat.p) (void)hipMemset(d_sat.p, 0, 4);
}

void F5::steps(int U, int N, int k0, int nsteps, const int* lens) {
    MI_REQUIRE(k0 >= 0 && nsteps >= 0 && k0 + nsteps <= cfg.nfe - 1, "f5: step range exceeds the NFE grid");
    MI_REQUIRE(!lens || lens == d_len.p, "f5: ragged steps read the handle's length table");
    if (!use_graph || prof_mask() != 0 || nsteps < 2) { steps_eager(U, N, k0, nsteps, lens); return; }
    if (graph_epoch != option_epoch()) { drop_graphs(); graph_epoch = option_epoch(); }
    GraphEntry& e = graphs[{U, N, k0, nsteps, lens ? 1 : 0}];
    if (e.exec) { MI_HIP(hipGraphLaunch(e.exec, stream)); return; }
    if (e.uses++ == 0) { steps_eager(U, N, k0, nsteps, lens); return; }
    hipGraph_t graph = nullptr;
    MI_HIP(hipStreamBeginCapture(stream, hipStreamCaptureModeThreadLocal));
    try {
        steps_eager(U, N, k0, nsteps, lens);
    } catch (...) {
        (void)hipStreamEndCapture(stream, &graph);
        if (graph) (void)hipGraphDestroy(graph);
        throw;
    }
    MI_HIP(hipStreamEndCapture(stream, &graph));
    hipError_t err = hipGraphInstantiate(&e.exec, graph, nullptr, nullptr, 0);
    (void)hipGraphDestroy(graph);
    if (err != hipSuccess) { e.exec = nullptr; use_graph = false; steps_eager(U, N, k0, nsteps, lens); return; }
    MI_HIP(hipGraphLaunch(e.exec, stream));
}

int F5::ref_frames(long L) const {
    const int mel_pad = cfg.mel_type == 1 ? (cfg.n_fft - cfg.hop) / 2 : cfg.n_fft / 2;
    return (int)((L + 2 * mel_pad - cfg.n_fft) / cfg.hop) + 1;
}

const int* F5::set_lengths(int U, const int* lens) {
    h_len.assign(lens, lens + U);
    if ((size_t)U * 4 > d_len.bytes) { drop_graphs(); d_len.ensure((size_t)std::max(U, 8) * 4); }
    MI_HIP(hipMemcpyAsync(d_len.p, h_len.data(), (size_t)U * 4, hipMemcpyHostToDevice, stream));
    return d_len.as<int>();
}

void F5::zero_pad_rows_cond(int U, int Nmax, const int* lens) {
    const size_t cd = cfg.cond_dim(), M = cfg.mel;
    for (int u = 0; u < U; ++u) {
        const size_t n = (size_t)lens[u], pad = (size_t)(Nmax - lens[u]);
        if (pad == 0) continue;
        MI_HIP(hipMemsetAsync(d_noise.as<float>() + ((size_t)u * Nmax + n) * M, 0, pad * M * 4, stream));
        MI_HIP(hipMemsetAsync(d_cmt.as<float>() + ((size_t)u * Nmax + n) * cd, 0, pad * cd * 4, stream));
        MI_HIP(hipMemsetAsync(d_cmtd.as<float>() + ((size_t)u * Nmax + n) * cd, 0, pad * cd * 4, stream));
    }
}

void F5::preprocess_ragged(int U, const int16_t* audio, const long* L, const int32_t* text_ids, const int* T, const int* Ns, int Nmax,
                           const float* noise_in, uint64_t seed, int mem, int* R) {
    const size_t M = cfg.mel, cd = cfg.cond_dim();
    MI_HIP(hipSetDevice(device));
    ensure_workspace(U, Nmax);
    std::vector<long> a_off(U + 1, 0), t_off(U + 1, 0), n_off(U + 1, 0);
    for (int u = 0; u < U; ++u) { a_off[u + 1] = a_off[u] + L[u]; t_off[u + 1] = t_off[u] + T[u]; n_off[u + 1] = n_off[u] + Ns[u]; }
    const hipMemcpyKind d2d = hipMemcpyDeviceToDevice;
    for (int u = U - 1; u >= 0; --u) {
        const int N = Ns[u];
        R[u] = preprocess(1, audio + a_off[u], L[u], text_ids + t_off[u], T[u], N, noise_in ? noise_in + (size_t)n_off[u] * M : nullptr,
                          seed + (uint64_t)u, mem);
        if (u > 0) {
            MI_HIP(hipMemcpyAsync(d_noise.as<float>() + (size_t)u * Nmax * M, d_noise.p, (size_t)N * M * 4, d2d, stream));
            MI_HIP(hipMemcpyAsync(d_cmt.as<float>() + (size_t)u * Nmax * cd, d_cmt.p, (size_t)N * cd * 4, d2d, stream));
            MI_HIP(hipMemcpyAsync(d_cmtd.as<float>() + (size_t)u * Nmax * cd, d_cmtd.p, (size_t)N * cd * 4, d2d, stream));
        }
        MI_HIP(hipStreamSynchronize(stream));
        check_text_ids();
    }
    zero_pad_rows_cond(U, Nmax, Ns);
}

long F5::decode(const float* den, int U, int N, int R, float* out_f, int16_t* out_i) {
    const F5Cfg& c = cfg;
    const int F = N - R;
    MI_REQUIRE(R >= 0 && F >= 1, "f5_decode: max_duration leaves no generated frame");
    if (F == 1) return 0;
    hipStream_t s = stream;
    const int vd = c.vd, vi = c.vi, nf = c.n_fft, nb = c.nb();
    const long rows = (long)U * F;
    float* h = v_h.as<float>(); float* z = v_z.as<float>(); float* z2 = v_z2.as<float>();
    {
        ConvGemm g;
        g.dtype = MI_F32; g.x = den + (size_t)R * c.mel; g.w = v_embed.w.p; g.bias = v_embed.b.as<float>(); g.out = h;
        g.B = U; g.T_in = F; g.M = F; g.N = vd; g.Cin = c.mel; g.taps = 7; g.pad = 3;
        g.x_bstride = (long)N * c.mel; g.x_rstride = c.mel; g.out_bstride = (long)F * vd; g.out_rstride = vd;
        launch_conv_gemm(g, s);
    }
    launch_rownorm(NORM_L2, h, h, MI_F32, v_norm_w.as<float>(), v_norm_b.as<float>(), rows, vd, 0.f, s);
    for (auto& vbk : vblocks) {
        launch_dwconv7(h, z, vbk.dw_w.as<float>(), vbk.dw_b.as<float>(), U, F, vd, s);
        launch_rownorm(NORM_L2, z, z, MI_F32, vbk.n_w.as<float>(), vbk.n_b.as<float>(), rows, vd, 0.f, s);
        gemm(MI_F32, z, (long)F * vd, vd, vd, vbk.pw1, z2, MI_F32, (long)F * vi, vi, U, F, ACT_GELU_ERF);
        gemm(MI_F32, z2, (long)F * vi, vi, vi, vbk.pw2, h, MI_F32, (long)F * vd, vd, U, F, ACT_NONE, h);
    }
    launch_rownorm(NORM_L2, h, z, MI_F32, v_fnorm_w.as<float>(), v_fnorm_b.as<float>(), rows, vd, 0.f, s);
    gemm(MI_F32, z, (long)F * vd, vd, vd, v_head, v_s.p, MI_F32, (long)F * 2 * nb, 2 * nb, U, F);
    launch_vocos_head(v_s.as<float>(), v_c.as<float>(), rows, nb, istft.k, s);
    gemm(MI_F32, v_c.p, (long)F * istft.k, istft.k, istft.k, istft, v_fr.p, MI_F32, (long)F * nf, nf, U, F);
    launch_istft_ola(v_fr.as<float>(), wsi.as<float>(), U, F, nf, c.hop, out_f, out_i, s);
    return (long)(F - 1) * c.hop;
}

}
```

text-to-speech-tts-onnx_amd/csrc/f5_kernels.h:

```cpp
#pragma once
#include "common.h"

namespace mi {

enum { NORM_LN_MOD = 0, NORM_LN_AFFINE = 1, NORM_L2 = 2 };
void launch_rownorm(int mode, const float* x, void* y, int out_dtype, const float* a, const float* b, long rows, int D,
                    float eps, hipStream_t s);
void launch_rownorm_len(int mode, const float* x, void* y, int out_dtype, const float* a, const float* b, int items, int Fmax, int D,
                        float eps, const int* lens, const long* offs, hipStream_t s);
void launch_rownorm_x3p(const float* x, void* planes, const float* a, const float* b, long rows, int D, float eps, hipStream_t s,
                        int np = 3, int* sat = nullptr);
void launch_ln_prologue(const float* x, void* aout, int a_dtype, int np, float* stats, const float* scale, long rows, int D, int* sat,
                        hipStream_t s);
void launch_ln_finalize(const float* partials, float* fin, long rows, int D, float eps, hipStream_t s);
void launch_ln_gather(const float* mod, long mod_ld, long col_scale, long col_shift, float* G, float* S, int steps, int D, hipStream_t s);
void launch_cast_to_f32(const void* src, int dtype, float* dst, long n, hipStream_t s);
void launch_absmax(const float* x, long n, unsigned* out_bits, hipStream_t s);
void launch_dwconv7(const float* x, float* y, const float* w, const float* bias, int B, int T, int C, hipStream_t s);
void launch_grn(float* y, float* ss_scratch, const float* gamma, const float* beta, int B, int T, int C, hipStream_t s);
void launch_text_gather(const int* ids, const float* emb, const float* pos, float* out, int U, int N, int C, hipStream_t s);
void launch_text_ids(const int32_t* in, int* out, int U, int T, int N, int vocab, int* err, hipStream_t s);
void launch_mask_rows(const int* ids, float* x, int V, int N, int C, hipStream_t s);
void launch_copy2d(const float* src, long lds_, void* dst, long ldd, long rows, int cols, int out_dtype, hipStream_t s);
void launch_pad_reflect(const int16_t* a, float* out, int U, long L, int half, hipStream_t s);
void launch_spec_mag(const float* spec, float* mag, int F, int nb, int ldm, float eps, hipStream_t s);
void launch_logmel(const float* melraw, float* cmt, float* cmtd, int U, int N, int R, int M, int ld, hipStream_t s);
void launch_vocos_head(const float* sp, float* c, long rows, int nb, int ldc, hipStream_t s);
void launch_istft_ola(const float* frames, const float* wsi, int U, int F, int nfft, int hop, float* out_f,
                      int16_t* out_i, hipStream_t s);
void launch_cat_noise(const float* noise, void* cat, int U, int N, int M, int ldc, int dtype, hipStream_t s);
void launch_cfg_update(float* noise, const float* pred, int U, int N, int M, float cfg, const float* dt, int k, hipStream_t s, int parts = 1);
void launch_cfg_update_len(float* noise, const float* pred, int U, int N, int M, float cfg, const float* dt, int k, const int* len,
                           hipStream_t s, int parts = 1);
void launch_zero_pad_rows(void* x, long row_bytes, int items, int N, const int* len, int per, hipStream_t s);
void launch_sum_parts(const float* in, float* out, long rows, int M, int parts, hipStream_t s);

struct AttnKvLayout {
    int kv_planes = 0;
    long k_ld = 0;
    long v_ld = 0;
    int v_rows = 0;
};
AttnKvLayout attention_kv_layout(int N, int dtype, bool caller_can_presplit_kv);
enum AttnForm {
    ATTN_F32 = 0, ATTN_F32_QK_X3 = 2, ATTN_X3F = 4, ATTN_X3F_BF16X3 = 6, ATTN_X3F_PAIRS = 8,
    ATTN_X3F_PAIRS_SLICED = 10,
    ATTN_F16 = 11, ATTN_F16_REF = 13, ATTN_BF16 = 15, ATTN_FORMS = 17
};
constexpr int ATTN_TILE = 128, ATTN_TILE_SPLIT = 64, ATTN_STAGE = 64, ATTN_MAX_SLICES = 4;
constexpr long ATTN_SLOT_GROUP = 32 * 64 + 64 * 2, ATTN_SLOT_SPLIT = 2 * ATTN_SLOT_GROUP, ATTN_SLOT = 4 * ATTN_SLOT_GROUP;
constexpr long ATTN_WS_TILES = 2048;
struct AttnPlan {
    AttnKvLayout kv;
    bool o_planes = false;
    int form = ATTN_F32;
    bool varlen = false;
    int BH = 0, H = 0, N = 0, dtype = MI_F32;
    unsigned grid[3] = {1, 1, 1};
    int cut[3] = {0, 0, 0};
    int xmap = 0;
    float sscale = 1.f;
    const char* label = "";
};
AttnPlan attention_plan(int BH, int H, int N, int dtype, bool caller_can_presplit_kv, bool has_lens, float ref_fp16_scale, long ws_floats,
                        long cnt_n);
void launch_attention(const AttnPlan& plan, const void* q, const void* k, const void* v, void* o, void* o_planes, int o_np, float* ws,
                      int* cnt, const int* lens, hipStream_t s);

}
```

text-to-speech-tts-onnx_amd/csrc/f5_kernels.hip:

```cpp
#include <type_traits>
#include "wave_reduce.h"
#include "common.h"
#include "f5_kernels.h"
#include "x3_split.h"

namespace mi {


template <typename TO, int MAXV, bool LENS = false>
__global__ __launch_bounds__(256) void rownorm_kernel(const float* __restrict__ x, TO* __restrict__ y,
                                                      const float* __restrict__ a, const float* __restrict__ b,
                                                      long rows, int D, int mode, float eps, const int* lens = nullptr,
                                                      const long* offs = nullptr, int Fmax = 0) {
    const int lane = threadIdx.x & 63;
    const long row = (long)blockIdx.x * 4 + (threadIdx.x >> 6);
    if (row >= rows) return;
    const float* xr = x + row * D;
    if constexpr (LENS) {
        const int it = __builtin_amdgcn_readfirstlane((int)(row / Fmax)), t = (int)(row - (long)it * Fmax);
        if (t >= __builtin_amdgcn_readfirstlane(lens[it])) {
            TO* yz = y + row * D;
#pragma unroll
            for (int i = 0; i < MAXV; ++i) {
                const int c = (i * 64 + lane) * 4;
                if (c < D) {
                    if constexpr (sizeof(TO) == 4) *reinterpret_cast<float4*>(yz + c) = make_float4(0.f, 0.f, 0.f, 0.f);
                    else *reinterpret_cast<uint2*>(yz + c) = make_uint2(0, 0);
                }
            }
            return;
        }
        xr = x + (offs[it] + t) * D;
    }
    float4 v[MAXV], av[MAXV], bv[MAXV];
    float s = 0.f;
#pragma unroll
    for (int i = 0; i < MAXV; ++i) {
        const int c = (i * 64 + lane) * 4;
        v[i] = c < D ? *reinterpret_cast<const float4*>(xr + c) : make_float4(0, 0, 0, 0);
    }
#pragma unroll
    for (int i = 0; i < MAXV; ++i) {
        const int c = (i * 64 + lane) * 4, cc = c < D ? c : 0;
        av[i] = *reinterpret_cast<const float4*>(a + cc);
        bv[i] = *reinterpret_cast<const float4*>(b + cc);
    }
#pragma unroll
    for (int i = 0; i < MAXV; ++i) s += (v[i].x + v[i].y) + (v[i].z + v[i].w);
    float mean = 0.f, inv;
    if (mode == NORM_L2) {
        float q = 0.f;
#pragma unroll
        for (int i = 0; i < MAXV; ++i) q += v[i].x * v[i].x + v[i].y * v[i].y + v[i].z * v[i].z + v[i].w * v[i].w;
        inv = 1.0f / sqrtf(wave_sum(q));
    } else {
        mean = wave_sum(s) / (float)D;
        float q = 0.f;
#pragma unroll
        for (int i = 0; i < MAXV; ++i) {
            const int c = (i * 64 + lane) * 4;
            if (c < D) {
                const float d0 = v[i].x - mean, d1 = v[i].y - mean, d2 = v[i].z - mean, d3 = v[i].w - mean;
                q += d0 * d0 + d1 * d1 + d2 * d2 + d3 * d3;
            }
        }
        inv = 1.0f / sqrtf(wave_sum(q) / (float)D + eps);
    }
    TO* yr = y + row * D;
#pragma unroll
    for (int i = 0; i < MAXV; ++i) {
        const int c = (i * 64 + lane) * 4;
        if (c < D) {
            float o[4] = {v[i].x, v[i].y, v[i].z, v[i].w};
            const float aa[4] = {av[i].x, av[i].y, av[i].z, av[i].w}, bb[4] = {bv[i].x, bv[i].y, bv[i].z, bv[i].w};
#pragma unroll
            for (int k = 0; k < 4; ++k) {
                const float n = (o[k] - mean) * inv;
                o[k] = mode == NORM_LN_MOD ? n * (1.f + aa[k]) + bb[k] : n * aa[k] + bb[k];
            }
            if constexpr (sizeof(TO) == 4) {
                *reinterpret_cast<float4*>(yr + c) = make_float4(o[0], o[1], o[2], o[3]);
            } else {
                TO h[4] = {from_f32<TO>(o[0]), from_f32<TO>(o[1]), from_f32<TO>(o[2]), from_f32<TO>(o[3])};
                *reinterpret_cast<uint2*>(yr + c) = *reinterpret_cast<const uint2*>(h);
            }
        }
    }
}

template <int MAXP, int NP>
__global__ __launch_bounds__(256) void rownorm_x3p_kernel(const float* __restrict__ x, unsigned char* __restrict__ planes,
                                                          const float* __restrict__ a, const float* __restrict__ b,
                                                          long rows, int D, float eps, int* __restrict__ satp) {
    const int lane = threadIdx.x & 63;
    const long row = (long)blockIdx.x * 4 + (threadIdx.x >> 6);
    if (row >= rows) return;
    const float* xr = x + row * D;
    unsigned sat = 0;
    float4 v[MAXP][2], av[MAXP][2], bv[MAXP][2];
    float s = 0.f;
#pragma unroll
    for (int i = 0; i < MAXP; ++i) {
        const int c = (i * 64 + lane) * 8;
        const bool in = c < D;
        v[i][0] = in ? *reinterpret_cast<const float4*>(xr + c) : make_float4(0, 0, 0, 0);
        v[i][1] = in ? *reinterpret_cast<const float4*>(xr + c + 4) : make_float4(0, 0, 0, 0);
    }
#pragma unroll
    for (int i = 0; i < MAXP; ++i) {
        const int c = (i * 64 + lane) * 8, cc = c < D ? c : 0;
        av[i][0] = *reinterpret_cast<const float4*>(a + cc); av[i][1] = *reinterpret_cast<const float4*>(a + cc + 4);
        bv[i][0] = *reinterpret_cast<const float4*>(b + cc); bv[i][1] = *reinterpret_cast<const float4*>(b + cc + 4);
    }
#pragma unroll
    for (int i = 0; i < MAXP; ++i)
        s += ((v[i][0].x + v[i][0].y) + (v[i][0].z + v[i][0].w)) + ((v[i][1].x + v[i][1].y) + (v[i][1].z + v[i][1].w));
    const float mean = wave_sum(s) / (float)D;
    float q = 0.f;
#pragma unroll
    for (int i = 0; i < MAXP; ++i) {
        const int c = (i * 64 + lane) * 8;
        if (c < D) {
#pragma unroll
            for (int h = 0; h < 2; ++h) {
                const float d0 = v[i][h].x - mean, d1 = v[i][h].y - mean, d2 = v[i][h].z - mean, d3 = v[i][h].w - mean;
                q += d0 * d0 + d1 * d1 + d2 * d2 + d3 * d3;
            }
        }
    }
    const float inv = 1.0f / sqrtf(wave_sum(q) / (float)D + eps);
    const int nch = D >> 5;
#pragma unroll
    for (int i = 0; i < MAXP; ++i) {
        const int s8 = i * 64 + lane, c = s8 * 8;
        if (c < D) {
            float o[8] = {v[i][0].x, v[i][0].y, v[i][0].z, v[i][0].w, v[i][1].x, v[i][1].y, v[i][1].z, v[i][1].w};
            const float4 a0 = av[i][0], a1 = av[i][1], b0 = bv[i][0], b1 = bv[i][1];
            const float aa[8] = {a0.x, a0.y, a0.z, a0.w, a1.x, a1.y, a1.z, a1.w}, bb[8] = {b0.x, b0.y, b0.z, b0.w, b1.x, b1.y, b1.z, b1.w};
#pragma unroll
            for (int k = 0; k < 8; ++k) o[k] = (o[k] - mean) * inv * (1.f + aa[k]) + bb[k];
            u32x4 pl[NP];
            xnp_split8_sat<NP>(o, pl, sat);
            unsigned char* dst = planes + x3p_slot_offset(row, s8, nch, NP);
#pragma unroll
            for (int q = 0; q < NP; ++q) *reinterpret_cast<u32x4*>(dst + q * X3P_PLANE) = pl[q];
        }
    }
    if constexpr (NP == 2) sat_publish(satp, sat);
}

void launch_rownorm_x3p(const float* x, void* planes, const float* a, const float* b, long rows, int D, float eps, hipStream_t s, int np, int* sat) {
    MI_REQUIRE(D % 32 == 0 && D <= 2048, "rownorm_x3p: D must be whole 32-deep chunks and <= 2048");
    MI_REQUIRE(np == 2 || np == 3, "rownorm_x3p: 2 or 3 planes");
    dim3 grid((unsigned)((rows + 3) / 4));
    ProfScope ps(FAM_NORM, s, (double)rows * D * (4.0 + 2.0 * np), 8.0 * rows * D);
    prof_set_kernel(np == 3 ? "rownorm_x3p_kernel<3 planes>" : "rownorm_x3p_kernel<2 planes>", "", "");
// ... 353 lines not shown
    if (i >= (long)N * M) return;
    const int n = (int)(i / M), m = (int)(i - (long)n * M);
    const long u = blockIdx.y;
    melraw += u * R * M; cmt += u * N * ld; cmtd += u * N * ld;
    cmt[(long)n * ld + m] = n < R ? logf(fmaxf(melraw[(long)n * M + m], 1e-5f)) : 0.f;
    cmtd[(long)n * ld + m] = 0.f;
}
void launch_logmel(const float* melraw, float* cmt, float* cmtd, int U, int N, int R, int M, int ld, hipStream_t s) {
    const long n = (long)N * M;
    hipLaunchKernelGGL(logmel_kernel, dim3((unsigned)((n + 255) / 256), U), dim3(256), 0, s, melraw, cmt, cmtd, N, R, M, ld);
    MI_HIP(hipGetLastError());
}

__global__ __launch_bounds__(256) void vocos_head_kernel(const float* __restrict__ sp, float* __restrict__ c, long rows, int nb, int ldc) {
    const long i = (long)blockIdx.x * 256 + threadIdx.x;
    if (i >= rows * ldc) return;
    const long r = i / ldc;
    const int k = (int)(i - r * ldc);
    float v = 0.f;
    if (k < 2 * nb) {
        const int kk = k < nb ? k : k - nb;
        const float mag = fminf(expf(sp[r * 2 * nb + kk]), 100.0f);
        const float ph = sp[r * 2 * nb + nb + kk];
        v = k < nb ? mag * cosf(ph) : mag * sinf(ph);
    }
    c[i] = v;
}
void launch_vocos_head(const float* sp, float* c, long rows, int nb, int ldc, hipStream_t s) {
    const long n = rows * ldc;
    hipLaunchKernelGGL(vocos_head_kernel, dim3((unsigned)((n + 255) / 256)), dim3(256), 0, s, sp, c, rows, nb, ldc);
    MI_HIP(hipGetLastError());
}

__global__ __launch_bounds__(256) void istft_ola_kernel(const float* __restrict__ fr, const float* __restrict__ wsi,
                                                        int F, int nfft, int hop, float* __restrict__ out_f,
                                                        int16_t* __restrict__ out_i) {
    const long len = (long)(F - 1) * hop;
    const long i = (long)blockIdx.x * 256 + threadIdx.x;
    const int u = blockIdx.y;
    if (i >= len) return;
    const long t = i + nfft / 2;
    long f1 = t / hop;
    if (f1 > F - 1) f1 = F - 1;
    long f0 = (t - nfft + hop) / hop;
    if (t - nfft + 1 <= 0) f0 = 0;
    const float* fb = fr + (long)u * F * nfft;
    float acc = 0.f;
    for (long f = f0; f <= f1; ++f) acc += fb[f * nfft + (t - f * hop)];
    float v = acc * wsi[t];
    if (out_f) out_f[(long)u * len + i] = v;
    if (out_i) {
        v = fminf(fmaxf(v, -1.0f), 1.0f) * 32767.0f;
        out_i[(long)u * len + i] = (int16_t)v;
    }
}
void launch_istft_ola(const float* frames, const float* wsi, int U, int F, int nfft, int hop, float* out_f,
                      int16_t* out_i, hipStream_t s) {
    const long len = (long)(F - 1) * hop;
    if (len <= 0) return;
    hipLaunchKernelGGL(istft_ola_kernel, dim3((unsigned)((len + 255) / 256), U), dim3(256), 0, s, frames, wsi, F, nfft, hop, out_f, out_i);
    MI_HIP(hipGetLastError());
}

template <typename T>
__global__ __launch_bounds__(256) void cat_noise_kernel(const float* __restrict__ noise, T* __restrict__ cat, long UN, int M, int ldc, int N) {
    const long i = (long)blockIdx.x * 256 + threadIdx.x;
    if (i >= UN * M) return;
    const long un = i / M;
    const int m = (int)(i - un * M);
    const long u = un / N, n = un - u * N;
    const T v = from_f32<T>(noise[i]);
    cat[((2 * u) * N + n) * ldc + m] = v;
    cat[((2 * u + 1) * N + n) * ldc + m] = v;
}
void launch_cat_noise(const float* noise, void* cat, int U, int N, int M, int ldc, int dtype, hipStream_t s) {
    const long n = (long)U * N * M;
    dim3 grid((unsigned)((n + 255) / 256));
    if (dtype == MI_F32) hipLaunchKernelGGL(cat_noise_kernel<float>, grid, dim3(256), 0, s, noise, (float*)cat, (long)U * N, M, ldc, N);
    else if (dtype == MI_F16) hipLaunchKernelGGL(cat_noise_kernel<f16>, grid, dim3(256), 0, s, noise, (f16*)cat, (long)U * N, M, ldc, N);
    else hipLaunchKernelGGL(cat_noise_kernel<bf16>, grid, dim3(256), 0, s, noise, (bf16*)cat, (long)U * N, M, ldc, N);
    MI_HIP(hipGetLastError());
}

__global__ __launch_bounds__(256) void cfg_update_kernel(float* __restrict__ noise, const float* __restrict__ pred,
                                                         long NM, int M, int parts, long total, float cfg, const float* __restrict__ dt, int k) {
    const long i = (long)blockIdx.x * 256 + threadIdx.x;
    if (i >= total) return;
    const long u = i / NM, r = i - u * NM;
    const long n = r / M; const int m = (int)(r - n * M);
    const float* c = pred + ((2 * u) * NM + n * M) * parts + m;
    const float* un = c + NM * parts;
    float pc = c[0], pu = un[0];
    for (int q = 1; q < parts; ++q) { pc += c[(long)q * M]; pu += un[(long)q * M]; }
    noise[i] += (pc + (pc - pu) * cfg) * dt[k];
}
void launch_cfg_update(float* noise, const float* pred, int U, int N, int M, float cfg, const float* dt, int k, hipStream_t s, int parts) {
    const long total = (long)U * N * M;
    hipLaunchKernelGGL(cfg_update_kernel, dim3((unsigned)((total + 255) / 256)), dim3(256), 0, s, noise, pred, (long)N * M, M, parts, total, cfg, dt, k);
    MI_HIP(hipGetLastError());
}

__global__ __launch_bounds__(256) void cfg_update_len_kernel(float* __restrict__ noise, const float* __restrict__ pred,
                                                             long NM, int M, int parts, long total, float cfg, const float* __restrict__ dt,
                                                             int k, const int* __restrict__ len) {
    const long i = (long)blockIdx.x * 256 + threadIdx.x;
    if (i >= total) return;
    const long u = i / NM, r = i - u * NM;
    const long n = r / M; const int m = (int)(r - n * M);
    if (n >= len[u]) { noise[i] = 0.f; return; }
    const float* c = pred + ((2 * u) * NM + n * M) * parts + m;
    const float* un = c + NM * parts;
    float pc = c[0], pu = un[0];
    for (int q = 1; q < parts; ++q) { pc += c[(long)q * M]; pu += un[(long)q * M]; }
    noise[i] += (pc + (pc - pu) * cfg) * dt[k];
}
void launch_cfg_update_len(float* noise, const float* pred, int U, int N, int M, float cfg, const float* dt, int k, const int* len,
                           hipStream_t s, int parts) {
    const long total = (long)U * N * M;
    hipLaunchKernelGGL(cfg_update_len_kernel, dim3((unsigned)((total + 255) / 256)), dim3(256), 0, s, noise, pred, (long)N * M, M, parts,
                       total, cfg, dt, k, len);
    MI_HIP(hipGetLastError());
}

__global__ __launch_bounds__(256) void zero_pad_rows_kernel(uint4* __restrict__ x, int row_vec, int N, const int* __restrict__ len, int per) {
    const int item = (int)blockIdx.y, r0 = (int)blockIdx.x * 8;
    const int live = len[item / per];
    if (r0 + 8 <= live) return;
    const int first = r0 > live ? r0 : live, last = r0 + 8 < N ? r0 + 8 : N;
    uint4* base = x + (long)item * N * row_vec;
    for (long i = (long)first * row_vec + threadIdx.x; i < (long)last * row_vec; i += 256) base[i] = make_uint4(0, 0, 0, 0);
}
void launch_zero_pad_rows(void* x, long row_bytes, int items, int N, const int* len, int per, hipStream_t s) {
    MI_REQUIRE(row_bytes % 16 == 0 && items > 0 && N > 0 && per > 0, "zero_pad_rows: bad shape");
    hipLaunchKernelGGL(zero_pad_rows_kernel, dim3((unsigned)((N + 7) / 8), (unsigned)items), dim3(256), 0, s, (uint4*)x, (int)(row_bytes / 16),
                       N, len, per);
    MI_HIP(hipGetLastError());
}

__global__ __launch_bounds__(256) void sum_parts_kernel(const float* __restrict__ in, float* __restrict__ out, long total, int M, int parts) {
    const long i = (long)blockIdx.x * 256 + threadIdx.x;
    if (i >= total) return;
    const long row = i / M; const int m = (int)(i - row * M);
    const float* p = in + row * M * parts + m;
    float v = p[0];
    for (int q = 1; q < parts; ++q) v += p[(long)q * M];
    out[i] = v;
}
void launch_sum_parts(const float* in, float* out, long rows, int M, int parts, hipStream_t s) {
    const long total = rows * M;
    hipLaunchKernelGGL(sum_parts_kernel, dim3((unsigned)((total + 255) / 256)), dim3(256), 0, s, in, out, total, M, parts);
    MI_HIP(hipGetLastError());
}

}
```

text-to-speech-tts-onnx_amd/csrc/gemm_conv.hip:

```cpp
#include "common.h"
#include <mutex>
#include "mfma.h"
#include "gemm_epilogue.h"
#include "lds_dma.h"

namespace mi {

template <typename T, typename TO, int BM, int BN, int WGM, int WGN, int KC, bool LENS = false>
__global__ __launch_bounds__(256, 2) void conv_gemm_kernel(const ConvGemmDev p) {
    using MF = Mfma<T>;
    constexpr int KP = MF::KP;
    constexpr int VEC = 16 / (int)sizeof(T);
    constexpr int KV = KC / VEC;
    constexpr int RPP = 256 / KV;
    constexpr int AP = (BM + RPP - 1) / RPP, BP = (BN + RPP - 1) / RPP;
    constexpr int LDA = KC + (sizeof(T) == 4 ? 1 : 8);
    constexpr int WM = BM / WGM, WN = BN / WGN, TM = WM / 32, TN = WN / 32;
    static_assert(WGM * WGN == 4 && WM % 32 == 0 && WN % 32 == 0, "tile");
    static_assert(KC % (2 * KP) == 0, "KC");

    __shared__ __attribute__((aligned(16))) T smem[(BM + BN) * LDA];
    T* As = smem;
    T* Bs = smem + BM * LDA;

// ... 661 lines not shown
    const long chb = x3p_chunk_bytes(p.np);
    return (p.np == 2 || p.np == 3) && p.N % 128 == 0 && ((long)(p.M + 127) / 128) * nch * chb < 0x7fff0000L && ((long)p.N / 128) * nch * chb < 0x7fff0000L;
}

bool gemm_x3p_would_run(const ConvGemm& p) { return x3p_eligible(p) && p.B == 1 && p.G == 1; }

static bool lds_epi_for(const ConvGemm& p, int odt, bool use_x3) {
    if (!opt(OPT_GEMM_LDS_EPI)) return false;
    const int ch = 16 / (int)dtype_size(odt);
    const bool qkv_lds = p.epi == EPI_QKV_ROPE && p.head_dim == 64 && (dtype_size(odt) == 2 || use_x3) && p.G == 1 &&
                         (p.rows_per_item == 0 ? p.M : p.rows_per_item) >= 64 && ((uintptr_t)p.out % 16) == 0 &&
                         ((uintptr_t)p.out2 % 16) == 0;
    if (qkv_lds) return true;
    return p.epi == EPI_PLAIN && p.taps == 1 && p.N >= 1024 && p.N % ch == 0 && p.out_rstride % ch == 0 &&
           p.out_bstride % ch == 0 && ((uintptr_t)p.out % 16) == 0 && (!p.res || ((uintptr_t)p.res % 16) == 0);
}

bool gemm_x3p_can_write_planes(const ConvGemm& p) {
    return gemm_x3p_would_run(p) && p.epi == EPI_PLAIN && !p.res && !p.gate && !p.accumulate && p.alpha == 1.f && p.N % 32 == 0 &&
           lds_epi_for(p, MI_F32, true);
}

bool gemm_ln_fold_ok(const ConvGemm& p) {
    const int odt = p.out_dtype < 0 ? p.dtype : p.out_dtype;
    if (p.B != 1 || p.G != 1 || p.taps != 1 || p.pad != 0 || p.alpha != 1.f || p.accumulate || p.gate_bstride != 0 || p.N % 64 != 0 || p.M <= 128) return false;
    if (p.epi != EPI_PLAIN && p.epi != EPI_QKV_ROPE) return false;
    if (p.dtype == MI_F32) return gemm_x3p_would_run(p) && lds_epi_for(p, odt, true);
    if (!lds_epi_for(p, odt, false) || !opt(OPT_GEMM_USE_DMA) || p.Cin % 64 != 0 || p.N <= 64) return false;
    if (opt(OPT_GEMM_USE_DMA3) && p.Cin > opt(OPT_GEMM_DMA3_K_MIN)) return false;
    return true;
}

void launch_conv_gemm(const ConvGemm& p_in, hipStream_t s) {
    ConvGemm p = p_in;
    if (!p.lens && p.B > 1 && p.taps == 1 && p.G == 1 && p.pad == 0 && p.epi == EPI_PLAIN && p.M == p.T_in && p.gate_bstride == 0 &&
        p.x_bstride == (long)p.M * p.x_rstride && p.out_bstride == (long)p.M * p.out_rstride) {
        p.T_in = p.M = p.B * p.M; p.B = 1;
    }
    const int odt = p.out_dtype < 0 ? p.dtype : p.out_dtype;
    const bool split_plain = p.epi == EPI_PLAIN && p.gate_bstride == 0 && !p.out_planes && !p.accumulate;
    const bool split_qkv = p.epi == EPI_QKV_ROPE && p.rows_per_item >= 32 && !p.kv_planes && p.m_off == 0;
    if (!p.lens && opt(OPT_GEMM_ROW_SPLIT) != 0 && opt(OPT_GEMM_PH8) != 0 && dtype_size(p.dtype) == 2 && p.B == 1 && p.G == 1 && p.taps == 1 && p.pad == 0 &&
        (split_plain || split_qkv) && p.M == p.T_in && p.N % 256 == 0 && !p.xp) {
        const int cus = device_cus();
        const long ntn = p.N / 256;
        long gc = cus, t = ntn;
        while (t) { const long u = gc % t; gc = t; t = u; }
        const long rstep = cus / gc;
        const long r = (p.M / 256) / rstep * rstep;
        const long rem = p.M - 256 * r;
        const long rem_tiles = (rem + 255) / 256 * ntn;
        if (r >= 1 && rem > 0 && rem_tiles * 2 < cus && r * ntn >= opt(OPT_GEMM_PH8_MIN_TILES)) {
            ConvGemm a = p, b = p;
            a.M = a.T_in = (int)(256 * r);
            b.M = b.T_in = (int)rem;
            b.x = (const char*)p.x + (size_t)(256 * r) * p.x_rstride * dtype_size(p.dtype);
            if (split_qkv) b.m_off = (int)(256 * r);
            else {
                b.out = (char*)p.out + (size_t)(256 * r) * p.out_rstride * dtype_size(odt);
                if (p.res) b.res = (const char*)p.res + (size_t)(256 * r) * p.out_rstride * dtype_size(odt);
                if (p.ln_stats_in) b.ln_stats_in = p.ln_stats_in + (size_t)(256 * r) * (p.ln_final ? 1 : p.ln_dim / LN_BLK) * 2;
                if (p.ln_stats_out) {
                    b.ln_stats_out = p.ln_stats_out + (size_t)(256 * r) * (p.N / LN_BLK) * 2;
                    b.ln_out = (char*)p.ln_out + (size_t)(256 * r) * p.N * dtype_size(p.dtype);
                }
            }
            launch_conv_gemm(a, s);
            launch_conv_gemm(b, s);
            return;
        }
    }
    const int vec = 16 / (int)dtype_size(p.dtype);
    MI_REQUIRE(p.Cin % vec == 0, "conv_gemm: Cin must be a multiple of the 16-byte vector");
    MI_REQUIRE(p.x_rstride % vec == 0 && p.x_bstride % vec == 0 && p.x_goff % vec == 0, "conv_gemm: x strides");
    MI_REQUIRE(((uintptr_t)p.x % 16) == 0 && ((uintptr_t)p.w % 16) == 0, "conv_gemm: 16-byte alignment");
    MI_REQUIRE(odt == p.dtype || odt == MI_F32, "conv_gemm: out dtype");
    MI_REQUIRE(p.M > 0 && p.N > 0 && p.B > 0 && p.G > 0, "conv_gemm: empty problem");
    ConvGemmDev d;
    d.x = p.x; d.w = p.w; d.bias = p.bias; d.out = p.out; d.res = p.res; d.gate = p.gate;
    d.gate_bstride = p.gate_bstride;
    d.G = p.G; d.T_in = p.T_in; d.M = p.M; d.N = p.N; d.Cin = p.Cin; d.K = p.taps * p.Cin; d.dil = p.dil; d.pad = p.pad;
    d.x_bstride = p.x_bstride; d.x_rstride = p.x_rstride; d.out_bstride = p.out_bstride; d.out_rstride = p.out_rstride;
    d.x_goff = p.x_goff;
    d.act = p.act; d.alpha = p.alpha; d.accumulate = p.accumulate; d.epi = p.epi;
    d.u = p.u; d.Cout = p.Cout; d.padT = p.padT; d.T_out = p.T_out;
    d.rope_cos = p.rope_cos; d.rope_sin = p.rope_sin; d.rope_pack = p.rope_pack; d.heads = p.heads; d.head_dim = p.head_dim;
    d.out2 = p.out2; d.out3 = p.out3; d.v_ld = p.v_ld; d.Mb = p.rows_per_item; d.m_off = p.m_off;
    MI_REQUIRE(p.m_off == 0 || (p.epi == EPI_QKV_ROPE && p.rows_per_item >= 32), "conv_gemm: a row offset needs the flattened QKV epilogue");
    d.kv_planes = p.kv_planes; d.k_ld = p.k_ld; d.v_rows = p.kv_planes ? p.v_rows : 0;
    d.sk_ws = p.sk_ws; d.sk_flags = p.sk_flags; d.sk_slots = p.sk_slots;
    const bool use_x3p = x3p_eligible(p);
    const bool use_x3 = use_x3p || x3_eligible(p);
    d.w3 = use_x3 ? p.w3 : nullptr;
    d.xp = use_x3p ? p.xp : nullptr; d.w3p = use_x3p ? p.w3p : nullptr; d.np = p.np;
    d.out_planes = nullptr;
    if (p.out_planes) {
        MI_REQUIRE(use_x3p && p.epi == EPI_PLAIN && !p.res && !p.gate && !p.accumulate && p.alpha == 1.f && p.N % 32 == 0,
                   "conv_gemm: out_planes needs the panel-plane kernel and a plain bias + activation epilogue");
        d.out_planes = p.out_planes;
    }
    d.ln_scale = p.ln_scale; d.ln_out = p.ln_out; d.ln_stats_out = p.ln_stats_out; d.ln_out_np = p.ln_out_np;
    d.ln_stats_in = p.ln_stats_in; d.ln_p = p.ln_p; d.ln_c = p.ln_c; d.ln_dim = p.ln_dim; d.ln_eps = p.ln_eps; d.ln_final = p.ln_final;
    d.sat = p.sat;
    d.lens = p.lens; d.len_mul = p.len_mul; d.len_add = p.len_add;
    if (p.lens)
        MI_REQUIRE((p.epi == EPI_PLAIN || p.epi == EPI_CONVT) && !p.ln_stats_in && !p.ln_stats_out && !p.out_planes && !p.xp && !p.w3 &&
                       !p.gcp_w && p.G == 1 && !p.gate,
                   "conv_gemm: a launch with lengths is a plain or ConvTranspose1d convolution over padded slabs");
    if (p.ln_stats_in || p.ln_stats_out) {
        MI_REQUIRE(!(p.ln_stats_in && p.ln_stats_out), "conv_gemm: a launch is the producer OR the consumer of the AdaLN fold");
        MI_REQUIRE(p.B == 1 && p.G == 1 && p.taps == 1 && p.alpha == 1.f && !p.accumulate && p.gate_bstride == 0 && p.N % 64 == 0,
                   "conv_gemm: AdaLN fold needs a plain linear layer over one M axis");
        if (p.ln_stats_out)
            MI_REQUIRE(p.epi == EPI_PLAIN && odt == MI_F32 && p.res && p.ln_scale && p.ln_out && p.act == ACT_NONE && !p.out_planes &&
                           ((uintptr_t)p.ln_out % 16) == 0 && ((uintptr_t)p.ln_stats_out % 8) == 0 && ((uintptr_t)p.ln_scale % 16) == 0 &&
                           (p.dtype != MI_F32 || p.ln_out_np == p.np),
                       "conv_gemm: AdaLN fold producer: fp32 residual rows out, (1 + scale) and the next operand's buffer");
        else
            MI_REQUIRE(p.ln_p && p.ln_c && p.ln_dim >= 128 && p.ln_dim % 128 == 0 && !p.res && !p.gate && ((uintptr_t)p.ln_stats_in % 8) == 0 && (p.ln_final || ((uintptr_t)p.ln_stats_in % 16) == 0) &&
                           ((uintptr_t)p.ln_p % 16) == 0 && ((uintptr_t)p.ln_c % 16) == 0 && (odt != MI_F32 || p.epi == EPI_QKV_ROPE || p.out_planes),
                       "conv_gemm: AdaLN fold consumer: statistics, W(1 + scale) and W shift + b vectors");
    }
    d.tail_tiles = 0; d.tail_split = 1;
    d.use_buf = 0;
    {
        int dev = 0;
        MI_HIP(hipGetDevice(&dev));
        {
            static std::mutex zero_mu;
            std::lock_guard<std::mutex> lk(zero_mu);
            DevBuf& z = g_zero_page[dev & 15];
            if (!z.p) { z.ensure(4096); MI_HIP(hipMemset(z.p, 0, 4096)); MI_HIP(hipDeviceSynchronize()); }
            d.zero = z.p;
        }
        d.dbg = (int)env_int("MI355TTS_GEMM_DBG", 0);
        d.lds_epi = (!p.lens && lds_epi_for(p, odt, use_x3)) ? 1 : 0;
    }
    if (p.ln_stats_in || p.ln_stats_out)
        MI_REQUIRE(d.lds_epi && (p.dtype != MI_F32 || use_x3p), "conv_gemm: the AdaLN fold lives in the LDS-staged epilogues of linear_x3p / linear_ph8 / conv_gemm_dma (gemm_ln_fold_ok)");
    if (p.kv_planes) MI_REQUIRE(p.epi == EPI_QKV_ROPE && p.dtype == MI_F32 && d.lds_epi && p.v_ld > 0 && p.k_ld > 0 && p.v_ld % 8 == 0,
                                "conv_gemm: kv_planes needs the fp32 LDS-staged QKV epilogue and the padded key axes k_ld / v_ld");
    if (p.epi == EPI_CONVT) MI_REQUIRE(p.Cout > 0 && p.N == p.u * p.Cout, "conv_gemm: convT shape");
    if (p.epi == EPI_QKV_ROPE)
        MI_REQUIRE((p.rows_per_item == 0 || p.rows_per_item >= 32) && p.G == 1 && p.heads > 0 && p.head_dim % 2 == 0 && p.N == 3 * p.heads * p.head_dim && p.N % 32 == 0 &&
                       p.rope_cos && p.rope_sin && p.out2 && p.out3, "conv_gemm: qkv-rope epilogue arguments");

    const double esz = (double)dtype_size(p.dtype), osz = (double)dtype_size(odt);
    const double rows_out = p.epi == EPI_CONVT ? (double)p.T_out : (double)p.M;
    const double ncols = p.epi == EPI_CONVT ? (double)p.Cout : (double)p.N * p.G;
    double bytes = (double)p.B * p.T_in * (double)p.Cin * p.G * esz + (double)p.G * p.N * d.K * esz +
                   (double)p.B * rows_out * ncols * osz * (1.0 + (p.res ? 1.0 : 0.0) + (p.accumulate ? 1.0 : 0.0));
    double flops = 2.0 * p.B * p.G * (double)p.M * p.N * d.K;
    ProfScope ps(FAM_CONV_GEMM, s, bytes, flops);

    if (!p.lens && p.dtype == MI_F32 && opt_x3() != 0 && opt_n64_pairs() != 0 && opt_gconv() != 0 && opt(OPT_GEMM_USE_DMA) && launch_gconv_pairs(p, s)) return;
    if (!p.lens && p.dtype != MI_F32 && p.gcp_w && opt(OPT_GEMM_USE_DMA) && launch_gconv16(p, s)) return;
    if (p.lens) {
        MI_REQUIRE(odt == p.dtype, "conv_gemm: a launch with lengths writes the engine dtype");
        if (p.dtype == MI_F32) dispatch_tiles<float, float, true>(d, p.B, s);
        else if (p.dtype == MI_F16) dispatch_tiles<f16, f16, true>(d, p.B, s);
        else dispatch_tiles<bf16, bf16, true>(d, p.B, s);
        return;
    }
    if (p.dtype == MI_F32) {
        dispatch_tiles<float, float, false>(d, p.B, s);
    } else if (p.dtype == MI_F16) {
        if (odt == MI_F32) dispatch_tiles<f16, float, false>(d, p.B, s);
        else dispatch_tiles<f16, f16, false>(d, p.B, s);
    } else {
        if (odt == MI_F32) dispatch_tiles<bf16, float, false>(d, p.B, s);
        else dispatch_tiles<bf16, bf16, false>(d, p.B, s);
    }
}

void SkWorkspace::ensure(int n_slots, hipStream_t s) {
    if (n_slots <= slots) return;
    ws.ensure((size_t)n_slots * 128 * 128 * 4);
    flags.ensure((size_t)n_slots * 4);
    MI_HIP(hipMemsetAsync(flags.p, 0, (size_t)n_slots * 4, s));
    MI_HIP(hipStreamSynchronize(s));
    slots = n_slots;
}

bool SkWorkspace::tripped() const {
    if (!flags.p || slots <= 0) return false;
    int v = 0;
    if (hipMemcpy(&v, (const int*)flags.p + slots - 1, 4, hipMemcpyDeviceToHost) != hipSuccess) return false;
    return v != 0;
}

void SkWorkspace::reset(hipStream_t s) {
    if (!flags.p || slots <= 0) return;
    (void)hipMemsetAsync(flags.p, 0, (size_t)slots * 4, s);
    (void)hipStreamSynchronize(s);
}

}
```

text-to-speech-tts-onnx_amd/mi355tts/f5.py:

```python
from __future__ import annotations

import ctypes as C
from typing import Optional

import numpy as np

from . import _lib
from .config import F5Config
from .weights import pack_f5


def _p(a):
    return None if a is None else a.ctypes.data


def ragged_layout(cfg: F5Config, audio_lens, text_lens, max_durations):
    L = [int(x) for x in audio_lens]
    T = [int(x) for x in text_lens]
    N = [int(x) for x in max_durations]
    if not L or len(T) != len(L) or len(N) != len(L):
        raise ValueError("ragged batch: audio_lens, text_lens and max_durations need one entry per utterance (at least one)")
    R, F, out = [], [], []
    for u, (l, t, n) in enumerate(zip(L, T, N)):
        if l < cfg.n_fft // 2 + 1 or cfg.ref_frames(l) < 1:
            raise ValueError(f"utterance {u}: prompt audio of {l} samples is shorter than one STFT frame")
        if t < 0:
            raise ValueError(f"utterance {u}: negative text length")
        r = cfg.ref_frames(l)
        if n < r + 1:
            raise ValueError(f"utterance {u}: max_duration {n} leaves no generated frame after {r} prompt frames")
        if n < t:
            raise ValueError(f"utterance {u}: max_duration {n} is shorter than the text ({t} ids)")
        if n > cfg.max_signal_length:
            raise ValueError(f"utterance {u}: max_duration {n} exceeds max_signal_length {cfg.max_signal_length}")
        R.append(r); F.append(n - r); out.append((n - r - 1) * cfg.hop_length)
    return R, F, out, max(N)


class F5Engine:
    def __init__(self, cfg: F5Config, state: Optional[dict] = None, *, blob: Optional[np.ndarray] = None,
                 blob_device=None, dtype: str = "f32", device: int = 0):
        self.cfg, self.dtype, self.device, self._h = cfg, dtype, device, None
        L = _lib.load()
        _lib.init(device)
        self._ci = np.asarray(cfg.to_int_array(), dtype=np.int32)
        self._cf = np.asarray(cfg.to_float_array(), dtype=np.float32)
        if blob_device is not None:
            import torch
            t = blob_device
            if not (t.is_cuda and t.dtype == torch.float32 and t.is_contiguous() and t.device.index == device):
                raise ValueError("blob_device must be a contiguous float32 CUDA tensor on the engine's device")
            expect = L.mi_f5_param_count(_lib.i32p(self._ci), len(self._ci), _lib.f32p(self._cf), len(self._cf))
            if expect != t.numel():
                raise _lib.MiError(f"weight blob has {t.numel()} floats, config needs {expect}")
            torch.cuda.current_stream(t.device).synchronize()
            self._h = L.mi_f5_create_mem(_lib.i32p(self._ci), len(self._ci), _lib.f32p(self._cf), len(self._cf),
                                         t.data_ptr(), t.numel(), _lib.DTYPES[dtype], device, _lib.MI_DEVICE)
            if not self._h:
                raise _lib.MiError("mi_f5_create_mem: " + L.mi_last_error().decode())
            return
        if blob is None:
            if state is None:
                raise ValueError("F5Engine needs an (unfolded, upstream-named) state dict or a packed blob")
            blob = pack_f5(cfg, state)
        blob = np.ascontiguousarray(blob, dtype=np.float32)
        self._ci = np.asarray(cfg.to_int_array(), dtype=np.int32)
        self._cf = np.asarray(cfg.to_float_array(), dtype=np.float32)
        expect = L.mi_f5_param_count(_lib.i32p(self._ci), len(self._ci), _lib.f32p(self._cf), len(self._cf))
        if expect != blob.size:
            raise _lib.MiError(f"weight blob has {blob.size} floats, config needs {expect}")
        self._h = L.mi_f5_create(_lib.i32p(self._ci), len(self._ci), _lib.f32p(self._cf), len(self._cf),
                                 _lib.f32p(blob), blob.size, _lib.DTYPES[dtype], device)
        if not self._h:
            raise _lib.MiError("mi_f5_create: " + L.mi_last_error().decode())

    def close(self):
        if getattr(self, "_h", None):
            _lib.load().mi_f5_destroy(self._h)
            self._h = None

    def __del__(self):
        try:
            self.close()
        except Exception:
            pass

    def info(self) -> dict:
        from .config import F32_ARITHMETIC_NAMES
        L = _lib.load()
        a = int(L.mi_f5_info(self._h, b"f32_arithmetic"))
        return {"f32_arithmetic": F32_ARITHMETIC_NAMES.get(a), "saturation_events": int(L.mi_f5_info(self._h, b"saturation_events")),
                "adaln_fold": bool(L.mi_f5_info(self._h, b"adaln_fold"))}

    def tables(self):
        te = np.empty((self.cfg.nfe_step, self.cfg.dim), np.float32)
        dt = np.empty((self.cfg.nfe_step - 1,), np.float32)
        _lib.check(_lib.load().mi_f5_tables(self._h, _lib.f32p(te), _lib.f32p(dt)), "mi_f5_tables")
        return te, dt

    def preprocess(self, audio, text_ids, max_duration, noise=None, seed: int = 9527):
        cfg = self.cfg
        audio = np.ascontiguousarray(np.asarray(audio).reshape(-1))
        if audio.dtype != np.int16:
            raise ValueError("audio must be int16")
        text_ids = np.ascontiguousarray(np.asarray(text_ids).reshape(-1), dtype=np.int32)
        N = int(np.asarray(max_duration).reshape(-1)[0])
        if noise is not None:
            noise = np.ascontiguousarray(noise, dtype=np.float32).reshape(N, cfg.mel_dim)
        out_noise = np.empty((1, N, cfg.mel_dim), np.float32)
        rc = np.empty((N, cfg.dim_head), np.float32)
        rs = np.empty((N, cfg.dim_head), np.float32)
        cd = cfg.mel_dim + cfg.text_dim
        cmt = np.empty((1, N, cd), np.float32)
        cmtd = np.empty((1, N, cd), np.float32)
        R = C.c_int64(0)
        _lib.check(_lib.load().mi_f5_preprocess(self._h, audio.ctypes.data, audio.size, text_ids.ctypes.data, text_ids.size,
                                                N, _p(noise), seed, out_noise.ctypes.data, rc.ctypes.data, rs.ctypes.data,
                                                cmt.ctypes.data, cmtd.ctypes.data, C.byref(R), _lib.MI_HOST),
                   "mi_f5_preprocess")
        H = cfg.heads
        cq = np.broadcast_to(rc[None, None], (2, H, N, cfg.dim_head))
        sq = np.broadcast_to(rs[None, None], (2, H, N, cfg.dim_head))
        return {"noise": out_noise, "rope_cos_q": cq, "rope_sin_q": sq, "rope_cos_k": cq.transpose(0, 1, 3, 2),
                "rope_sin_k": sq.transpose(0, 1, 3, 2), "cat_mel_text": cmt, "cat_mel_text_drop": cmtd,
                "ref_signal_len": np.int64(R.value)}

    def stft(self, audio):
        cfg = self.cfg
        audio = np.ascontiguousarray(np.asarray(audio).reshape(-1))
        if audio.dtype != np.int16:
            raise ValueError("audio must be int16")
        nb, R = cfg.n_fft // 2 + 1, audio.size // cfg.hop_length + 1
        spec = np.empty((R, 2 * nb), np.float32)
        _lib.check(_lib.load().mi_f5_stft(self._h, audio.ctypes.data, audio.size, spec.ctypes.data, _lib.MI_HOST), "mi_f5_stft")
        return np.ascontiguousarray(spec[:, :nb].T), np.ascontiguousarray(spec[:, nb:].T)

    def _cond(self, noise, cmt, cmtd):
        cfg = self.cfg
        noise = np.ascontiguousarray(noise, dtype=np.float32)
        if noise.ndim != 3 or noise.shape[2] != cfg.mel_dim:
            raise ValueError(f"noise must be (U, N, {cfg.mel_dim})")
        U, N, _ = noise.shape
        cd = cfg.mel_dim + cfg.text_dim
        cmt = np.ascontiguousarray(cmt, dtype=np.float32)
        cmtd = np.ascontiguousarray(cmtd, dtype=np.float32)
        if cmt.shape != (U, N, cd) or cmtd.shape != (U, N, cd):
            raise ValueError(f"cat_mel_text(_drop) must be ({U}, {N}, {cd})")
        return noise, cmt, cmtd, U, N

    def transformer_step(self, noise, cat_mel_text, cat_mel_text_drop, time_step, fuse: int = 1):
        noise, cmt, cmtd, U, N = self._cond(noise, cat_mel_text, cat_mel_text_drop)
        x = noise.copy()
        ts = np.asarray(time_step, dtype=np.int32).reshape(-1).copy()
        _lib.check(_lib.load().mi_f5_transformer_step(self._h, x.ctypes.data, cmt.ctypes.data, cmtd.ctypes.data, U, N,
                                                      _lib.i32p(ts), fuse, _lib.MI_HOST), "mi_f5_transformer_step")
        return x, ts

    def transformer_step_device(self, x, cat_mel_text, cat_mel_text_drop, k: int, fuse: int = 1) -> int:
        import torch
        for t in (x, cat_mel_text, cat_mel_text_drop):
            if not (t.is_cuda and t.dtype == torch.float32 and t.is_contiguous() and t.device.index == self.device):
                raise ValueError("operands must be contiguous float32 CUDA tensors on the engine's device")
        U, N, M = x.shape
        cd = self.cfg.mel_dim + self.cfg.text_dim
        if M != self.cfg.mel_dim or tuple(cat_mel_text.shape) != (U, N, cd) or tuple(cat_mel_text_drop.shape) != (U, N, cd):
            raise ValueError(f"x must be (U, N, {self.cfg.mel_dim}), cat_mel_text(_drop) (U, N, {cd})")
        torch.cuda.current_stream(x.device).synchronize()
        ts = C.c_int32(int(k))
        _lib.check(_lib.load().mi_f5_transformer_step(self._h, x.data_ptr(), cat_mel_text.data_ptr(), cat_mel_text_drop.data_ptr(),
                                                      U, N, C.byref(ts), int(fuse), _lib.MI_DEVICE), "mi_f5_transformer_step")
        return int(ts.value)

    def sample(self, noise, cat_mel_text, cat_mel_text_drop, k0: int = 0, n_steps: Optional[int] = None):
        noise, cmt, cmtd, U, N = self._cond(noise, cat_mel_text, cat_mel_text_drop)
        x = noise.copy()
        if n_steps is None:
            n_steps = self.cfg.nfe_step - 1 - k0
        _lib.check(_lib.load().mi_f5_sample(self._h, x.ctypes.data, cmt.ctypes.data, cmtd.ctypes.data, U, N, k0, n_steps,
                                            _lib.MI_HOST), "mi_f5_sample")
        return x

    def dit_eval(self, noise, cat_mel_text, cat_mel_text_drop, k: int):
        noise, cmt, cmtd, U, N = self._cond(noise, cat_mel_text, cat_mel_text_drop)
        pred = np.empty((2 * U, N, self.cfg.mel_dim), np.float32)
        _lib.check(_lib.load().mi_f5_dit_eval(self._h, noise.ctypes.data, cmt.ctypes.data, cmtd.ctypes.data, U, N, k,
                                              pred.ctypes.data, _lib.MI_HOST), "mi_f5_dit_eval")
        return pred

    def decode(self, denoised, ref_signal_len, return_float: bool = False):
        cfg = self.cfg
        den = np.ascontiguousarray(denoised, dtype=np.float32)
        if den.ndim != 3 or den.shape[2] != cfg.mel_dim:
            raise ValueError(f"denoised must be (U, N, {cfg.mel_dim})")
        U, N, _ = den.shape
        R = int(ref_signal_len)
        n = (N - R - 1) * cfg.hop_length
        if n < 0:
            raise ValueError("decode needs at least one generated frame")
        if n == 0:
            out0 = np.empty((U, 1, 0), np.int16)
            return (out0, np.empty((U, 1, 0), np.float32)) if return_float else out0
        out = np.empty((U, 1, n), np.int16)
        outf = np.empty((U, 1, n), np.float32) if return_float else None
        ln = C.c_int64(0)
        _lib.check(_lib.load().mi_f5_decode(self._h, den.ctypes.data, U, N, R, out.ctypes.data, _p(outf), C.byref(ln),
                                            _lib.MI_HOST), "mi_f5_decode")
        assert ln.value == n
        return (out, outf) if return_float else out

    def synthesize(self, audio, text_ids, max_duration, noise=None, seed: int = 9527):
        cfg = self.cfg
        audio = np.ascontiguousarray(np.atleast_2d(np.asarray(audio)))
        if audio.dtype != np.int16:
            raise ValueError("audio must be int16")
        text_ids = np.ascontiguousarray(np.atleast_2d(np.asarray(text_ids)), dtype=np.int32)
        U, Ln = audio.shape
        if text_ids.shape[0] != U:
            raise ValueError("audio / text_ids batch mismatch")
        N = int(max_duration)
        R = cfg.ref_frames(Ln)
        n = (N - R - 1) * cfg.hop_length
        if n < 0:
            raise ValueError("max_duration leaves no generated frames")
        if noise is not None:
            noise = np.ascontiguousarray(noise, dtype=np.float32).reshape(U, N, cfg.mel_dim)
        out = np.empty((U, 1, max(n, 0)), np.int16)
        ln = C.c_int64(0)
        _lib.check(_lib.load().mi_f5_synthesize(self._h, U, audio.ctypes.data, Ln, text_ids.ctypes.data, text_ids.shape[1],
                                                N, _p(noise), seed, out.ctypes.data, C.byref(ln), _lib.MI_HOST),
                   "mi_f5_synthesize")
        assert ln.value == n
        return out

    def synthesize_ragged(self, audios, text_ids, max_durations, noise=None, seed: int = 9527):
        cfg = self.cfg
        audios = [np.ascontiguousarray(np.asarray(a).reshape(-1)) for a in audios]
        if any(a.dtype != np.int16 for a in audios):
            raise ValueError("audio must be int16")
        ids = [np.ascontiguousarray(np.asarray(t).reshape(-1), dtype=np.int32) for t in text_ids]
        if len(ids) != len(audios) or len(max_durations) != len(audios):
            raise ValueError("audios / text_ids / max_durations batch mismatch")
        _, _, out_lens, _ = ragged_layout(cfg, [a.size for a in audios], [t.size for t in ids], max_durations)
        U = len(audios)
        N = [int(n) for n in max_durations]
        if noise is not None:
            if len(noise) != U:
# ... 159 lines not shown
```

Before: 43.02.

## Fuse DiT eval ends: split input projection and fuse final norm, proj_out and Euler update

The input projection is split into a per-call constant cond/text part, computed once per call, and a per-step noise part that reads pre-split fp16 planes. At the tail, a new seam kernel fuses the final AdaLN norm, proj_out on MFMA, the CFG/Euler update and writing the next step's noise planes. This removes per-step cat copies, redundant GEMM work over constant columns, and several kernel launches. It adds complexity, extra weight images and buffers, and fallback paths, and it only applies with F32, two planes and the AdaLN fold.

```diff
diff --git a/text-to-speech-tts-onnx_amd/csrc/capi.hip b/text-to-speech-tts-onnx_amd/csrc/capi.hip
--- a/text-to-speech-tts-onnx_amd/csrc/capi.hip
+++ b/text-to-speech-tts-onnx_amd/csrc/capi.hip
@@ -298,6 +298,7 @@
         if (k == "f32_arithmetic") v = e.dtype != MI_F32 ? -1 : !gemm_x3_enabled() ? ARITH_NATIVE : (gemm_x3p_enabled() ? e.np : ARITH_BF16X3);
         else if (k == "saturation_events") v = e.sat_events;
         else if (k == "adaln_fold") v = (e.fold_built && e.cfg.ln_fold != 0) ? 1 : 0;
+        else if (k == "eval_ends") v = e.eval_ends;
         else if (k == "attn_v_rows") v = attention_kv_layout(0, e.dtype, true).v_rows;
         else MI_REQUIRE(false, "mi_f5_info: unknown key");
     });
diff --git a/text-to-speech-tts-onnx_amd/csrc/common.h b/text-to-speech-tts-onnx_amd/csrc/common.h
--- a/text-to-speech-tts-onnx_amd/csrc/common.h
+++ b/text-to-speech-tts-onnx_amd/csrc/common.h
@@ -145,6 +145,7 @@
     int ln_final = 0;
     int* sat = nullptr;
     const int* lens = nullptr; int len_mul = 1, len_add = 0;
+    const char* prof_label = nullptr;
 };
 constexpr int LN_BLK = 32;
 void launch_conv_gemm(const ConvGemm& p, hipStream_t s);
diff --git a/text-to-speech-tts-onnx_amd/csrc/f5.h b/text-to-speech-tts-onnx_amd/csrc/f5.h
--- a/text-to-speech-tts-onnx_amd/csrc/f5.h
+++ b/text-to-speech-tts-onnx_amd/csrc/f5.h
@@ -34,6 +34,12 @@
     const float* pred_rows(int U, int N);
     int cat_pad = 0;
     int cat_ld() const { return cfg.cat_dim() + cat_pad; }
+    int eval_ends = 0;
+    Lin in_proj_x, in_proj_ct;
+    DevBuf Cproj, Axp, w_out_frag;
+    bool pred_is_rows = false;
+    int xk() const { return (cfg.mel + 31) / 32 * 32; }
+    bool ends_ready() const { return eval_ends && dtype == MI_F32 && np == 2 && fold_built && cfg.ln_fold != 0 && in_proj_x.w3p.p && Cproj.p && Axp.p; }
     struct Block { Lin qkv, o, ff1, ff2; };
     std::vector<Block> blocks;
     DevBuf mod;
@@ -90,14 +96,14 @@
     ~F5();
     void ensure_workspace(int U, int N);
     void gemm(int dt, const void* x, long xb, long xr, int K, const Lin& L, void* out, int odt, long ob, long orr,
-              int B, int M, int act = ACT_NONE, const void* res = nullptr, const float* gate = nullptr);
+              int B, int M, int act = ACT_NONE, const void* res = nullptr, const float* gate = nullptr, const char* prof_label = nullptr);
     int preprocess(int U, const int16_t* audio, long L, const int32_t* text_ids, int T, int N,
                    const float* noise_in, uint64_t seed, int mem);
     void stft(const int16_t* audio_dev, int U, long L, int pad = -1);
     void check_text_ids();
     void load_cond(const float* noise, const float* cmt, const float* cmtd, int U, int N, int mem);
     void build_cat_cond(int U, int N);
-    void dit_eval(int U, int N, int k, const int* lens = nullptr);
+    int dit_eval(int U, int N, int k, const int* lens = nullptr, int loop = 0);
     void steps(int U, int N, int k0, int nsteps, const int* lens = nullptr);
     DevBuf d_len;
     std::vector<int> h_len;
diff --git a/text-to-speech-tts-onnx_amd/csrc/f5.hip b/text-to-speech-tts-onnx_amd/csrc/f5.hip
--- a/text-to-speech-tts-onnx_amd/csrc/f5.hip
+++ b/text-to-speech-tts-onnx_amd/csrc/f5.hip
@@ -82,6 +82,7 @@
     MI_HIP(hipMemsetAsync(d_sat.p, 0, 64, s));
     const int d = c.dim, td = c.text_dim, ff = c.ff(), ti = td * c.conv_mult, cin = c.cat_dim();
     if (dt == MI_F32 && !env_first_is("MI355TTS_CAT_PAD", '0')) cat_pad = rup(cin, 64) - cin;
+    if (dt == MI_F32) eval_ends = (int)std::min<long>(std::max<long>(env_int("MI355TTS_EVAL_ENDS", 1), 0), 2);
     const float* p = w;
     auto take = [&](size_t n) { const float* r = p; p += n; return r; };
     BlobReader R(mem, s);
@@ -152,6 +153,18 @@
             std::vector<float> wp((size_t)d * kp, 0.f);
             for (int o = 0; o < d; ++o) std::copy(hw + (size_t)o * cin, hw + (size_t)(o + 1) * cin, wp.begin() + (size_t)o * kp);
             up_lin(in_proj, wp.data(), hb, d, kp, dt, s);
+        }
+        if (eval_ends) {
+            const int kp = cat_ld(), kx = xk();
+            const float* hw = R.host(pw, (size_t)d * cin); const float* hb = R.host(pb, d);
+            std::vector<float> wx((size_t)d * kx, 0.f), wc((size_t)d * kp, 0.f);
+            for (int o = 0; o < d; ++o) {
+                std::copy(hw + (size_t)o * cin, hw + (size_t)o * cin + c.mel, wx.begin() + (size_t)o * kx);
+                std::copy(hw + (size_t)o * cin + c.mel, hw + (size_t)(o + 1) * cin, wc.begin() + (size_t)o * kp + c.mel);
+            }
+            up_lin(in_proj_x, wx.data(), nullptr, d, kx, dt, s);
+            up_lin(in_proj_ct, wc.data(), hb, d, kp, dt, s);
+            MI_HIP(hipStreamSynchronize(s));
         }
         const int cg = d / c.pos_g;
         const size_t gw = (size_t)d * cg * c.pos_k;
@@ -240,11 +253,27 @@
         MI_HIP(hipStreamSynchronize(s));
         fold_built = true;
     }
+    if (eval_ends && !fold_built) {
+        eval_ends = 0;
+        for (Lin* L : {&in_proj_x, &in_proj_ct}) { L->w.release(); L->b.release(); L->w3p.release(); }
+    }
     {
         const float* mw = take((size_t)2 * d * d); const float* mb = take((size_t)2 * d);
         mod_gemm(mw, mb, 2 * d, (long)c.depth * 6 * d);
         const float* pw = take((size_t)c.mel * d); const float* pb = take(c.mel);
         put_lin(R, proj_out, pw, pb, c.mel, d, dt);
+        if (eval_ends == 1) {
+            bool ok = step_seam_supported(d, c.mel);
+            if (ok) {
+                w_out_frag.ensure(seam_wout_bytes(c.mel, d));
+                seam_split_wout(proj_out.w.as<float>(), w_out_frag.p, c.mel, d, d_sat.as<int>() + 2, s);
+                int flag = 0;
+                MI_HIP(hipMemcpyAsync(&flag, d_sat.as<int>() + 2, 4, hipMemcpyDeviceToHost, s));
+                MI_HIP(hipStreamSynchronize(s));
+                ok = flag == 0;
+            }
+            if (!ok) { w_out_frag.release(); eval_ends = 2; }
+        }
         {
             const int parts = (int)env_int("MI355TTS_PROJ_PARTS", 4);
             if (dt == MI_F32 && parts > 1 && parts <= 8 && d % (parts * 32) == 0) {
@@ -405,6 +434,7 @@
     for (Block& bk : blocks)
         for (Lin* L : {&bk.qkv, &bk.o, &bk.ff1, &bk.ff2}) build_planes(L);
     build_planes(&in_proj);
+    if (eval_ends) { build_planes(&in_proj_x); build_planes(&in_proj_ct); }
     if (ws_U > 0) {
         const long rows = (long)2 * ws_U * ws_N;
         Ap.ensure((size_t)x3p_bytes(rows, cfg.dim, np)); Ap2.ensure((size_t)x3p_bytes(rows, ap2_cols(), np)); ApN.ensure((size_t)x3p_bytes(rows, cfg.dim, np));
@@ -468,7 +498,13 @@
     d_cmtd.ensure((size_t)Um * Nm * c.cond_dim() * 4);
     if (rows * cat_ld() * es > cat.bytes) {
         cat.ensure(rows * cat_ld() * es);
-        if (cat_ld() != c.cat_dim()) MI_HIP(hipMemsetAsync(cat.p, 0, cat.bytes, stream));
+        if (cat_ld() != c.cat_dim() || eval_ends) MI_HIP(hipMemsetAsync(cat.p, 0, cat.bytes, stream));
+    }
+    if (eval_ends) {
+        Cproj.ensure(rows * c.dim * 4);
+        const size_t xb = (size_t)x3p_bytes((long)rows, xk(), 2);
+        if (xb > Axp.bytes) { Axp.ensure(xb); MI_HIP(hipMemsetAsync(Axp.p, 0, Axp.bytes, stream)); }
+        pred_sum.ensure(rows * c.mel * 4);
     }
     h32.ensure(rows * c.dim * 4); hT.ensure(rows * c.dim * es); c1.ensure(rows * c.dim * es);
     X.ensure(rows * c.dim * 4); Ub.ensure(rows * c.dim * es);
@@ -500,8 +536,9 @@
 }
 
 void F5::gemm(int dt, const void* x, long xb, long xr, int K, const Lin& L, void* out, int odt, long ob, long orr, int B,
-              int M, int act, const void* res, const float* gate) {
+              int M, int act, const void* res, const float* gate, const char* prof_label) {
     ConvGemm g;
+    g.prof_label = prof_label;
     g.dtype = dt; g.out_dtype = odt; g.x = x; g.w = L.w.p; g.w3 = L.w3.p; g.bias = L.b.p ? L.b.as<float>() : nullptr; g.out = out;
     g.res = res; g.gate = gate; g.gate_bstride = 0;
     g.B = B; g.T_in = M; g.M = M; g.N = L.n; g.Cin = K; g.taps = 1;
@@ -655,17 +692,36 @@
             char* dst = (char*)cat.p + ((size_t)(2 * u + br) * N * ld + c.mel) * es;
             launch_copy2d(src, cd, dst, ld, N, cd, dtype, stream);
         }
-}
-
-void F5::dit_eval(int U, int N, int k, const int* lens) {
+    if (ends_ready() && in_proj.w3p.p) gemm(dtype, cat.p, (long)N * ld, ld, ld, in_proj_ct, Cproj.p, MI_F32, (long)N * c.dim, c.dim, 2 * U, N, ACT_NONE, nullptr, nullptr,
+                                            "input projection: cond | text part, once per call");
+}
+
+int F5::dit_eval(int U, int N, int k, const int* lens, int loop) {
     const F5Cfg& c = cfg;
     MI_REQUIRE(k >= 0 && k < c.nfe, "f5: time step out of range");
     hipStream_t s = stream;
     const int B = 2 * U, d = c.dim, ld = cat_ld(), ff = c.ff(), H = c.heads, D = c.dim_head;
     const long rows = (long)B * N;
     const float* modk = mod.as<float>() + (size_t)k * mod_ld;
-    launch_cat_noise(d_noise.as<float>(), cat.p, U, N, c.mel, ld, dtype, s);
-    gemm(dtype, cat.p, (long)N * ld, ld, ld, in_proj, h32.p, MI_F32, (long)N * d, d, B, N);
+    pred_is_rows = false;
+    ConvGemm gx;
+    bool ends = false;
+    if (ends_ready() && in_proj.w3p.p) {
+        gx.dtype = dtype; gx.out_dtype = MI_F32; gx.x = Ub.p; gx.w = in_proj_x.w.p; gx.out = h32.p; gx.res = Cproj.p;
+        gx.B = 1; gx.T_in = (int)rows; gx.M = (int)rows; gx.N = d; gx.Cin = xk(); gx.taps = 1;
+        gx.x_bstride = rows * xk(); gx.x_rstride = xk(); gx.out_bstride = rows * d; gx.out_rstride = d;
+        gx.sat = d_sat.as<int>(); gx.xp = Axp.p; gx.w3p = in_proj_x.w3p.p; gx.np = np;
+        sk.attach(gx);
+        ends = gemm_x3p_would_run(gx);
+    }
+    if (ends) {
+        if (loop < 2)
+            launch_x_planes(d_noise.as<float>(), nullptr, Axp.p, U, N, c.mel, xk(), 1, 0.f, nullptr, 0, nullptr, d_sat.as<int>(), s);
+        launch_conv_gemm(gx, s);
+    } else {
+        launch_cat_noise(d_noise.as<float>(), cat.p, U, N, c.mel, ld, dtype, s);
+        gemm(dtype, cat.p, (long)N * ld, ld, ld, in_proj, h32.p, MI_F32, (long)N * d, d, B, N);
+    }
     const void* hin = h32.p;
     if (dtype != MI_F32) { launch_copy2d(h32.as<float>(), d, hT.p, d, rows, d, dtype, s); hin = hT.p; }
     const long row_bytes = (long)d * (long)dtype_size(dtype);
@@ -792,6 +848,20 @@
         gemm(dtype, Hff.p, (long)N * ff, ff, ff, bk.ff2, X.p, MI_F32, (long)N * d, d, B, N, ACT_NONE, X.p, m + 5 * d);
     }
     const float* mf = modk + (size_t)c.depth * 6 * d;
+    if (ends && eval_ends == 1 && w_out_frag.p) {
+        StepSeam a;
+        a.x = X.as<float>(); a.scale = mf; a.shift = mf + d; a.eps = 1e-6f; a.wfrag = w_out_frag.p; a.bias = proj_out.b.as<float>();
+        a.U = U; a.N = N; a.D = d; a.M = c.mel; a.sat = d_sat.as<int>();
+        if (loop) {
+            a.noise = d_noise.as<float>(); a.cfg = c.cfg_strength; a.dt = delta_t.as<float>(); a.k = k; a.len = lens;
+            a.planes = Axp.p; a.xk = xk();
+        } else {
+            a.pred = pred_sum.as<float>();
+            pred_is_rows = true;
+        }
+        launch_step_seam(a, s);
+        return 2;
+    }
     launch_rownorm(NORM_LN_MOD, X.as<float>(), Ub.p, dtype, mf, mf + d, rows, d, 1e-6f, s);
     if (proj_parts > 1) {
         ConvGemm g;
@@ -802,9 +872,11 @@
         launch_conv_gemm(g, s);
     } else
         gemm(dtype, Ub.p, (long)N * d, d, d, proj_out, pred.p, MI_F32, (long)N * c.mel, c.mel, B, N);
+    return ends ? 1 : 0;
 }
 
 const float* F5::pred_rows(int U, int N) {
+    if (pred_is_rows) return pred_sum.as<float>();
     if (proj_parts <= 1) return pred.as<float>();
     launch_sum_parts(pred.as<float>(), pred_sum.as<float>(), (long)2 * U * N, cfg.mel, proj_parts, stream);
     return pred_sum.as<float>();
@@ -812,8 +884,12 @@
 
 void F5::steps_eager(int U, int N, int k0, int nsteps, const int* lens) {
     for (int k = k0; k < k0 + nsteps; ++k) {
-        dit_eval(U, N, k, lens);
-        if (lens)
+        const int left = dit_eval(U, N, k, lens, k == k0 ? 1 : 2);
+        if (left == 2) continue;
+        if (left == 1)
+            launch_x_planes(d_noise.as<float>(), pred.as<float>(), Axp.p, U, N, cfg.mel, xk(), proj_parts, cfg.cfg_strength, delta_t.as<float>(),
+                            k, lens, d_sat.as<int>(), stream);
+        else if (lens)
             launch_cfg_update_len(d_noise.as<float>(), pred.as<float>(), U, N, cfg.mel, cfg.cfg_strength, delta_t.as<float>(), k, lens, stream,
                                   proj_parts);
         else
diff --git a/text-to-speech-tts-onnx_amd/csrc/f5_kernels.h b/text-to-speech-tts-onnx_amd/csrc/f5_kernels.h
--- a/text-to-speech-tts-onnx_amd/csrc/f5_kernels.h
+++ b/text-to-speech-tts-onnx_amd/csrc/f5_kernels.h
@@ -35,6 +35,23 @@
 void launch_zero_pad_rows(void* x, long row_bytes, int items, int N, const int* len, int per, hipStream_t s);
 void launch_sum_parts(const float* in, float* out, long rows, int M, int parts, hipStream_t s);
 
+void launch_x_planes(float* noise, const float* pred, void* planes, int U, int N, int M, int xk, int parts, float cfg, const float* dt,
+                     int k, const int* len, int* sat, hipStream_t s);
+size_t seam_wout_bytes(int M, int D);
+void seam_split_wout(const float* w, void* frag, int M, int D, int* sat, hipStream_t s);
+bool step_seam_supported(int D, int M);
+struct StepSeam {
+    const float* x = nullptr;
+    const float* scale = nullptr; const float* shift = nullptr; float eps = 1e-6f;
+    const void* wfrag = nullptr; const float* bias = nullptr;
+    int U = 0, N = 0, D = 0, M = 0;
+    float* pred = nullptr;
+    float* noise = nullptr; float cfg = 0.f; const float* dt = nullptr; int k = 0; const int* len = nullptr;
+    void* planes = nullptr; int xk = 0;
+    int* sat = nullptr;
+};
+void launch_step_seam(const StepSeam& a, hipStream_t s);
+
 struct AttnKvLayout {
     int kv_planes = 0;
     long k_ld = 0;
diff --git a/text-to-speech-tts-onnx_amd/csrc/f5_kernels.hip b/text-to-speech-tts-onnx_amd/csrc/f5_kernels.hip
--- a/text-to-speech-tts-onnx_amd/csrc/f5_kernels.hip
+++ b/text-to-speech-tts-onnx_amd/csrc/f5_kernels.hip
@@ -2,6 +2,7 @@
 #include "wave_reduce.h"
 #include "common.h"
 #include "f5_kernels.h"
+#include "mfma.h"
 #include "x3_split.h"
 
 namespace mi {
@@ -661,4 +662,251 @@
     MI_HIP(hipGetLastError());
 }
 
-}
+__global__ __launch_bounds__(256) void f5_x_planes_kernel(float* __restrict__ noise, const float* __restrict__ pred,
+                                                          unsigned char* __restrict__ planes, long total, int N, int M, int s8n, int parts,
+                                                          float cfg, const float* __restrict__ dt, int k, const int* __restrict__ len,
+                                                          int* __restrict__ satp) {
+    const long idx = (long)blockIdx.x * 256 + threadIdx.x;
+    if (idx >= total) return;
+    const long un = idx / s8n;
+    const int s8 = (int)(idx - un * s8n);
+    const long u = un / N, n = un - u * N;
+    const long NM = (long)N * M;
+    const bool dead = len && n >= len[u];
+    float v[8];
+#pragma unroll
+    for (int j = 0; j < 8; ++j) {
+        const int m = s8 * 8 + j;
+        float x = 0.f;
+        if (m < M) {
+            const long i = un * M + m;
+            x = noise[i];
+            if (pred) {
+                if (dead) x = 0.f;
+                else {
+                    const float* c = pred + ((2 * u) * NM + n * M) * parts + m;
+                    const float* un_ = c + NM * parts;
+                    float pc = c[0], pu = un_[0];
+                    for (int q = 1; q < parts; ++q) { pc += c[(long)q * M]; pu += un_[(long)q * M]; }
+                    x += (pc + (pc - pu) * cfg) * dt[k];
+                }
+                noise[i] = x;
+            }
+        }
+        v[j] = x;
+    }
+    u32x4 pl[2];
+    unsigned sat = 0;
+    xnp_split8_sat<2>(v, pl, sat);
+    const long r0 = (2 * u) * N + n;
+#pragma unroll
+    for (int br = 0; br < 2; ++br) {
+        unsigned char* dst = planes + x3p_slot_offset(r0 + (long)br * N, s8, s8n >> 2, 2);
+        *reinterpret_cast<u32x4*>(dst) = pl[0];
+        *reinterpret_cast<u32x4*>(dst + X3P_PLANE) = pl[1];
+    }
+    sat_publish(satp, sat);
+}
+void launch_x_planes(float* noise, const float* pred, void* planes, int U, int N, int M, int xk, int parts, float cfg, const float* dt,
+                     int k, const int* len, int* sat, hipStream_t s) {
+    MI_REQUIRE(xk % 32 == 0 && xk >= M && U > 0 && N > 0, "x_planes: K must be whole 32-deep chunks");
+    const long total = (long)U * N * (xk / 8);
+    ProfScope ps(FAM_OTHER, s, (double)U * N * (M * 4.0 * (pred ? 2 + 2 * parts : 1) + xk * 8.0), pred ? 5.0 * U * N * M : 0.0);
+    prof_set_kernel("f5_x_planes_kernel", "", "");
+    prof_kernel_suffix(pred ? " (CFG / Euler update + planes of x)" : " (planes of x)");
+    hipLaunchKernelGGL(f5_x_planes_kernel, dim3((unsigned)((total + 255) / 256)), dim3(256), 0, s, noise, pred, (unsigned char*)planes, total, N,
+                       M, xk / 8, parts, cfg, dt, k, len, sat);
+    MI_HIP(hipGetLastError());
+}
+
+constexpr int SEAM_ROWS = 16, SEAM_FRAMES = 8, SEAM_NT_MAX = 8, SEAM_D_MAX = 1024;
+__global__ __launch_bounds__(256) void f5_seam_split_wout_kernel(const float* __restrict__ w, unsigned char* __restrict__ frag, int M, int D,
+                                                                 int NT, long total, int* __restrict__ satp) {
+    const long idx = (long)blockIdx.x * 256 + threadIdx.x;
+    if (idx >= total) return;
+    const int lane = (int)(idx & 63);
+    const long t = idx >> 6;
+    const int ks = (int)(t / NT), nt = (int)(t - (long)ks * NT);
+    const int n = nt * 16 + (lane & 15), k0 = ks * 32 + 8 * (lane >> 4);
+    float v[8];
+#pragma unroll
+    for (int j = 0; j < 8; ++j) v[j] = n < M ? w[(long)n * D + k0 + j] : 0.f;
+    u32x4 pl[2];
+    unsigned sat = 0;
+    xnp_split8_sat<2>(v, pl, sat);
+    unsigned char* dst = frag + t * 2048 + lane * 16;
+    *reinterpret_cast<u32x4*>(dst) = pl[0];
+    *reinterpret_cast<u32x4*>(dst + 1024) = pl[1];
+    sat_publish(satp, sat);
+}
+size_t seam_wout_bytes(int M, int D) { return (size_t)(D / 32) * ((M + 15) / 16) * 2048; }
+bool step_seam_supported(int D, int M) { return D % 128 == 0 && D <= SEAM_D_MAX && M >= 1 && (M + 15) / 16 <= SEAM_NT_MAX; }
+void seam_split_wout(const float* w, void* frag, int M, int D, int* sat, hipStream_t s) {
+    MI_REQUIRE(step_seam_supported(D, M), "seam_split_wout: shape");
+    const int NT = (M + 15) / 16;
+    const long total = (long)(D / 32) * NT * 64;
+    hipLaunchKernelGGL(f5_seam_split_wout_kernel, dim3((unsigned)((total + 255) / 256)), dim3(256), 0, s, w, (unsigned char*)frag, M, D, NT, total, sat);
+    MI_HIP(hipGetLastError());
+}
+
+__global__ __launch_bounds__(256) void f5_step_seam_kernel(const StepSeam a) {
+    __shared__ __attribute__((aligned(16))) unsigned char smem[SEAM_ROWS * SEAM_D_MAX * 4];
+    (void)smem;
+#if defined(__HIP_DEVICE_COMPILE__)
+    typedef float f32x4 __attribute__((ext_vector_type(4)));
+    const int tid = threadIdx.x, lane = tid & 63;
+    const int wave = __builtin_amdgcn_readfirstlane(tid >> 6);
+    const int u = blockIdx.y, n0 = blockIdx.x * SEAM_FRAMES;
+    const int D = a.D, N = a.N, M = a.M;
+    const int plane_bytes = SEAM_ROWS * D * 2;
+    unsigned sat = 0;
+    constexpr int MAXP = SEAM_D_MAX / 512;
+#pragma unroll
+    for (int rr = 0; rr < 4; ++rr) {
+        const int row = wave * 4 + rr;
+        const int n = n0 + (row >> 1);
+        const bool live = n < N;
+        const float* xr = a.x + ((long)(2 * u + (row & 1)) * N + (live ? n : 0)) * D;
+        float4 v[MAXP][2], av[MAXP][2], bv[MAXP][2];
+        float s = 0.f;
+#pragma unroll
+        for (int i = 0; i < MAXP; ++i) {
+            const int c = (i * 64 + lane) * 8;
+            const bool in = live && c < D;
+            v[i][0] = in ? *reinterpret_cast<const float4*>(xr + c) : make_float4(0, 0, 0, 0);
+            v[i][1] = in ? *reinterpret_cast<const float4*>(xr + c + 4) : make_float4(0, 0, 0, 0);
+            const int cc = c < D ? c : 0;
+            av[i][0] = *reinterpret_cast<const float4*>(a.scale + cc); av[i][1] = *reinterpret_cast<const float4*>(a.scale + cc + 4);
+            bv[i][0] = *reinterpret_cast<const float4*>(a.shift + cc); bv[i][1] = *reinterpret_cast<const float4*>(a.shift + cc + 4);
+        }
+#pragma unroll
+        for (int i = 0; i < MAXP; ++i)
+            s += ((v[i][0].x + v[i][0].y) + (v[i][0].z + v[i][0].w)) + ((v[i][1].x + v[i][1].y) + (v[i][1].z + v[i][1].w));
+        const float mean = wave_sum(s) / (float)D;
+        float q = 0.f;
+#pragma unroll
+        for (int i = 0; i < MAXP; ++i) {
+            const int c = (i * 64 + lane) * 8;
+            if (c < D) {
+#pragma unroll
+                for (int h = 0; h < 2; ++h) {
+                    const float d0 = v[i][h].x - mean, d1 = v[i][h].y - mean, d2 = v[i][h].z - mean, d3 = v[i][h].w - mean;
+                    q += d0 * d0 + d1 * d1 + d2 * d2 + d3 * d3;
+                }
+            }
+        }
+        const float inv = 1.0f / sqrtf(wave_sum(q) / (float)D + a.eps);
+#pragma unroll
+        for (int i = 0; i < MAXP; ++i) {
+            const int s8 = i * 64 + lane, c = s8 * 8;
+            if (c < D) {
+                float o[8] = {v[i][0].x, v[i][0].y, v[i][0].z, v[i][0].w, v[i][1].x, v[i][1].y, v[i][1].z, v[i][1].w};
+                const float4 a0 = av[i][0], a1 = av[i][1], b0 = bv[i][0], b1 = bv[i][1];
+                const float aa[8] = {a0.x, a0.y, a0.z, a0.w, a1.x, a1.y, a1.z, a1.w}, bb[8] = {b0.x, b0.y, b0.z, b0.w, b1.x, b1.y, b1.z, b1.w};
+#pragma unroll
+                for (int k = 0; k < 8; ++k) o[k] = live ? (o[k] - mean) * inv * (1.f + aa[k]) + bb[k] : 0.f;
+                u32x4 pl[2];
+                xnp_split8_sat<2>(o, pl, sat);
+                unsigned char* dst = smem + s8 * 256 + ((row ^ (s8 & 15)) << 4);
+                *reinterpret_cast<u32x4*>(dst) = pl[0];
+                *reinterpret_cast<u32x4*>(dst + plane_bytes) = pl[1];
+            }
+        }
+    }
+    __syncthreads();
+    const int NT = (M + 15) >> 4;
+    const int nks = D >> 5, kq = nks >> 2;
+    f32x4 acc0[SEAM_NT_MAX], acc1[SEAM_NT_MAX];
+#pragma unroll
+    for (int j = 0; j < SEAM_NT_MAX; ++j) { acc0[j] = f32x4{0.f, 0.f, 0.f, 0.f}; acc1[j] = f32x4{0.f, 0.f, 0.f, 0.f}; }
+    const unsigned char* wf = (const unsigned char*)a.wfrag + lane * 16;
+#pragma unroll 2
+    for (int ks = wave * kq; ks < (wave + 1) * kq; ++ks) {
+        const int s8 = ks * 4 + (lane >> 4);
+        const unsigned char* ap = smem + s8 * 256 + (((lane & 15) ^ (s8 & 15)) << 4);
+        const f16x8 a_hi = *reinterpret_cast<const f16x8*>(ap), a_lo = *reinterpret_cast<const f16x8*>(ap + plane_bytes);
+        const unsigned char* bp = wf + (long)ks * NT * 2048;
+#pragma unroll
+        for (int j = 0; j < SEAM_NT_MAX; ++j) {
+            if (j < NT) {
+                const f16x8 b_hi = *reinterpret_cast<const f16x8*>(bp + j * 2048), b_lo = *reinterpret_cast<const f16x8*>(bp + j * 2048 + 1024);
+                acc1[j] = __builtin_amdgcn_mfma_f32_16x16x32_f16(a_lo, b_hi, acc1[j], 0, 0, 0);
+                acc0[j] = __builtin_amdgcn_mfma_f32_16x16x32_f16(a_hi, b_hi, acc0[j], 0, 0, 0);
+                acc1[j] = __builtin_amdgcn_mfma_f32_16x16x32_f16(a_hi, b_lo, acc1[j], 0, 0, 0);
+            }
+        }
+    }
+    __syncthreads();
+    f32x4* red = reinterpret_cast<f32x4*>(smem);
+    float* xs = reinterpret_cast<float*>(smem + 4 * SEAM_NT_MAX * 64 * 16);
+#pragma unroll
+    for (int j = 0; j < SEAM_NT_MAX; ++j)
+        if (j < NT) {
+            f32x4 t;
+#pragma unroll
+            for (int r = 0; r < 4; ++r) t[r] = __builtin_fmaf(acc1[j][r], 0x1p-11f, acc0[j][r]);
+            red[(wave * SEAM_NT_MAX + j) * 64 + lane] = t;
+        }
+    __syncthreads();
+    const float step = a.noise ? a.dt[a.k] : 0.f;
+    for (int it = tid; it < NT * 64; it += 256) {
+        const int j = it >> 6, l = it & 63;
+        f32x4 p = red[j * 64 + l];
+#pragma unroll
+        for (int w = 1; w < 4; ++w) { const f32x4 t = red[(w * SEAM_NT_MAX + j) * 64 + l]; p[0] += t[0]; p[1] += t[1]; p[2] += t[2]; p[3] += t[3]; }
+        const int m = j * 16 + (l & 15);
+        const bool col = m < M;
+        const float bm = col ? a.bias[m] : 0.f;
+#pragma unroll
+        for (int fr = 0; fr < 2; ++fr) {
+            const int f = 2 * (l >> 4) + fr, n = n0 + f;
+            const float pc = p[2 * fr] + bm, pu = p[2 * fr + 1] + bm;
+            if (a.pred && col && n < N) {
+                a.pred[((long)(2 * u) * N + n) * M + m] = pc;
+                a.pred[((long)(2 * u + 1) * N + n) * M + m] = pu;
+            }
+            if (a.noise) {
+                float x = 0.f;
+                if (col && n < N) {
+                    const long i = ((long)u * N + n) * M + m;
+                    if (!(a.len && n >= a.len[u])) x = a.noise[i] + (pc + (pc - pu) * a.cfg) * step;
+                    a.noise[i] = x;
+                }
+                xs[f * (NT * 16) + m] = x;
+            }
+        }
+    }
+    if (a.planes) {
+        __syncthreads();
+        const int s8n = a.xk >> 3;
+        for (int it = tid; it < SEAM_FRAMES * s8n; it += 256) {
+            const int f = it / s8n, s8 = it - f * s8n, n = n0 + f;
+            if (n >= N) continue;
+            float v[8];
+#pragma unroll
+            for (int q = 0; q < 8; ++q) { const int m = s8 * 8 + q; v[q] = m < M ? xs[f * (NT * 16) + m] : 0.f; }
+            u32x4 pl[2];
+            xnp_split8_sat<2>(v, pl, sat);
+#pragma unroll
+            for (int br = 0; br < 2; ++br) {
+                unsigned char* dst = (unsigned char*)a.planes + x3p_slot_offset((long)(2 * u + br) * N + n, s8, s8n >> 2, 2);
+                *reinterpret_cast<u32x4*>(dst) = pl[0];
+                *reinterpret_cast<u32x4*>(dst + X3P_PLANE) = pl[1];
+            }
+        }
+    }
+    sat_publish(a.sat, sat);
+#endif
+}
+void launch_step_seam(const StepSeam& a, hipStream_t s) {
+    MI_REQUIRE(step_seam_supported(a.D, a.M) && a.U > 0 && a.N > 0 && a.x && a.wfrag && a.bias && a.scale && a.shift, "step_seam: shape");
+    MI_REQUIRE((a.pred || a.noise) && (!a.noise || a.dt) && (!a.planes || (a.noise && a.xk % 32 == 0 && a.xk >= a.M)), "step_seam: outputs");
+    const double rows = 2.0 * a.U * a.N;
+    ProfScope ps(FAM_NORM, s, rows * (a.D * 4.0 + a.M * 4.0 + (a.planes ? a.xk * 4.0 : 0.0)), rows * a.D * (8.0 + 2.0 * a.M));
+    prof_set_kernel("f5_step_seam_kernel", "", "");
+    prof_kernel_suffix(a.pred ? " (AdaLN-final + proj_out -> pred rows)" : " (AdaLN-final + proj_out + CFG / Euler update + planes of x)");
+    hipLaunchKernelGGL(f5_step_seam_kernel, dim3((unsigned)((a.N + SEAM_FRAMES - 1) / SEAM_FRAMES), (unsigned)a.U), dim3(256), 0, s, a);
+    MI_HIP(hipGetLastError());
+}
+
+}
diff --git a/text-to-speech-tts-onnx_amd/csrc/gemm_conv.hip b/text-to-speech-tts-onnx_amd/csrc/gemm_conv.hip
--- a/text-to-speech-tts-onnx_amd/csrc/gemm_conv.hip
+++ b/text-to-speech-tts-onnx_amd/csrc/gemm_conv.hip
@@ -837,6 +837,7 @@
                    (double)p.B * rows_out * ncols * osz * (1.0 + (p.res ? 1.0 : 0.0) + (p.accumulate ? 1.0 : 0.0));
     double flops = 2.0 * p.B * p.G * (double)p.M * p.N * d.K;
     ProfScope ps(FAM_CONV_GEMM, s, bytes, flops);
+    struct Relabel { const char* l; ~Relabel() { if (l) prof_set_kernel(l, "", ""); } } relabel{p.prof_label};
 
     if (!p.lens && p.dtype == MI_F32 && opt_x3() != 0 && opt_n64_pairs() != 0 && opt_gconv() != 0 && opt(OPT_GEMM_USE_DMA) && launch_gconv_pairs(p, s)) return;
     if (!p.lens && p.dtype != MI_F32 && p.gcp_w && opt(OPT_GEMM_USE_DMA) && launch_gconv16(p, s)) return;
diff --git a/text-to-speech-tts-onnx_amd/mi355tts/f5.py b/text-to-speech-tts-onnx_amd/mi355tts/f5.py
--- a/text-to-speech-tts-onnx_amd/mi355tts/f5.py
+++ b/text-to-speech-tts-onnx_amd/mi355tts/f5.py
@@ -92,6 +92,9 @@
         return {"f32_arithmetic": F32_ARITHMETIC_NAMES.get(a), "saturation_events": int(L.mi_f5_info(self._h, b"saturation_events")),
                 "adaln_fold": bool(L.mi_f5_info(self._h, b"adaln_fold"))}
 
+    def eval_ends(self) -> int:
+        return int(_lib.load().mi_f5_info(self._h, b"eval_ends"))
+
     def tables(self):
         te = np.empty((self.cfg.nfe_step, self.cfg.dim), np.float32)
         dt = np.empty((self.cfg.nfe_step - 1,), np.float32)
```

Result: no change. 42.99, median of 3 (-0.1%).
